# sine2pi/ASR-model

Measured on AMD Instinct MI355X. Metric: audio-sec/sec fwd+bwd on 30s@16kHz LibriSpeech-shaped clips (whole job, all GPUs), higher is better.
Workload: dtype bf16; 1 GPU; tiny (BASELINE configs[1]): log-mel + 4 enc/4 dec d=384 h=6 fwd+bwd, 32 x 30 s clips per GPU, T=256; model=tiny, global_batch=32, seq_len=3001, text_len=256, pitch_frames=3001, parallelism=dp1

## Files before the change

### asr-model_amd/asrx/gemm.py

```python
from __future__ import annotations

import torch

from . import lib, prec, probe

ACT = {"none": 0, "gelu": 1, "silu": 2, "sigmoid": 3, "relu": 4}


BF16 = torch.bfloat16


def is_bf16(t) -> bool:
    return t is not None and t.dtype == BF16


def gemm(A, B, C, *, M, N, K, lda, ldb, ldc, a_kc=True, b_kc=True, batch=1, sA=0, sB=0, sC=0,
         bias=None, Z=None, alpha=1.0, beta=0.0, act="none", conv_a=False, conv_b=False,
         conv_F=0, conv_C=0, splitk=1, precision=None):
    lib.require_gpu(A, B, C)
    if is_bf16(A) or is_bf16(B) or is_bf16(C):
        raise RuntimeError("asrx_gemm takes fp32 operands; bf16-stored activations go through the wide GEMM")
    p = prec.get() if precision is None else precision
    e0 = probe.begin("gemm")
    lib.call("asrx_gemm", p, lib.ptr(A), lda, sA, int(a_kc), int(conv_a), lib.ptr(B), ldb, sB,
# ... 237 lines not shown


def gemm_wn_rows(A, Wb, C, *, M, N, K, lda, ldc, mtiles, bias=None, alpha=1.0, beta=0.0):
    return gemm_wn(A, Wb, C, M=M, N=N, K=K, lda=lda, ldc=ldc, bias=bias, alpha=alpha, beta=beta, mtiles=mtiles)


def row_tiles(next_i, layer, L, M, device=None):
    n = int(lib.load().asrx_row_tiles_max(M))
    dev = device if device is not None else next_i.device
    tl = torch.empty(n, dtype=torch.int32, device=dev)
    cnt = torch.empty(1, dtype=torch.int32, device=dev)
    lib.call("asrx_row_tiles", lib.ptr(next_i), layer, L, M, lib.ptr(tl), lib.ptr(cnt), lib.stream())
    return tl, cnt


def linear_fwd(x, W, b=None, act="none", out=None, preact=None, wbf=None, mtiles=None, out_bf16=False):
    x2 = _rows(x)
    if not x2.is_contiguous():
        x2 = x2.contiguous()
    M, K = x2.shape
    N = W.shape[0]
    wide = use_wide(K)
    if is_bf16(x2) and not wide:
        x2 = x2.float()
    odt = BF16 if (out_bf16 and wide and N % 4 == 0) else torch.float32
    y = out if out is not None else torch.empty(*x.shape[:-1], N, device=x.device, dtype=odt)
    if wide and mtiles is not None and act == "none" and preact is None:
        gemm_wn_rows(x2, weight_bf16(W) if wbf is None else wbf, y, M=M, N=N, K=K, lda=K, ldc=N, bias=b,
                     mtiles=mtiles)
    elif use_wide(K):
        gemm_wn(x2, weight_bf16(W) if wbf is None else wbf, y, M=M, N=N, K=K, lda=K, ldc=N, bias=b, act=act,
                Z=preact)
    else:
        gemm(x2, W, y, M=M, N=N, K=K, lda=K, ldb=K, ldc=N, a_kc=True, b_kc=True, bias=b, act=act,
             Z=preact)
    return y


def linear_rot_fwd(x, W, b, m, tab, L, hd, scale, preact=None):
    x2 = _rows(x)
    if not x2.is_contiguous():
        x2 = x2.contiguous()
    M, K = x2.shape
    N = W.shape[0]
    Wb = weight_bf16(W)
    y = torch.empty(*x.shape[:-1], N, device=x.device)
    nj = _nj(M, N)
    ab = int(is_bf16(x2))
    lib.require_gpu(x2, Wb, y, m, tab)
    e0 = probe.begin("gemm")
    lib.call("asrx_gemm_wn_rot", lib.ptr(x2), ab, K, lib.ptr(Wb), Wb.stride(0), lib.ptr(y), lib.ptr(preact), N,
             lib.ptr(b), lib.ptr(m), lib.ptr(tab), L, hd, float(scale), M, N, K, nj, lib.stream())
    probe.end("gemm", e0, 2.0 * M * N * K, ("wn", M, N, K, nj, 0, "rot", preact is not None, False, ab, 0, -1))
    return y


def linear_dgrad(dy, W, out=None, beta=0.0, mtiles=None):
    """dx = dy @ W for dy (..., N), W (N, K); mtiles as in linear_fwd."""
    d2 = _rows(dy)
    if not d2.is_contiguous():
        d2 = d2.contiguous()
    M, N = d2.shape
    K = W.shape[1]
    dx = out if out is not None else torch.empty(*dy.shape[:-1], K, device=dy.device, dtype=torch.float32)
    if use_wide(N) and mtiles is not None:
        gemm_wn_rows(d2, weight_bf16(W, trans=True), dx, M=M, N=K, K=N, lda=N, ldc=K, beta=beta, mtiles=mtiles)
    elif use_wide(N):
        gemm_wn(d2, weight_bf16(W, trans=True), dx, M=M, N=K, K=N, lda=N, ldc=K, beta=beta)
    else:
        gemm(d2, W, dx, M=M, N=K, K=N, lda=N, ldb=K, ldc=K, a_kc=True, b_kc=False, beta=beta)
    return dx


def _splitk_for(m_rows: int, tiles: int) -> int:
    want = max(1, 512 // max(tiles, 1))
    return int(max(1, min(want, m_rows // 256)))


FUSED_BIAS_GRAD = True
BIAS_CHECK = None


def _staged_f32_dy(A, lda, x2, M, K, rows):
    if is_bf16(x2):
        return None if (M % 4 or K % 8 or lda % 4 or x2.stride(0) != K or A.data_ptr() % 16) else 1
    tiles = ((M + 127) // 128) * ((K + 127) // 128)
    ok4 = M % 4 == 0 and K % 4 == 0 and lda % 4 == 0 and A.data_ptr() % 16 == 0 and x2.data_ptr() % 16 == 0
    if prec.get() == prec.PREC_BF16 and ok4 and x2.stride(0) == K and (tiles <= 9 or rows <= 16384
                                                                        or (rows <= 50000 and tiles <= 72)):
        return 0
    return None


def _wgrad(A, lda, x2, out, M, K, rows, db=None):
    tiles = ((M + 127) // 128) * ((K + 127) // 128)
    sk = _splitk_for(rows, tiles)

    def staged(a_bf16, b_bf16, name, *tag):
        lib.require_gpu(A, x2, out)
        e0 = probe.begin("gemm")
        if db is not None and not FUSED_BIAS_GRAD:
            staged_db, db_ = db, None
        else:
            staged_db, db_ = None, db
        if db_ is not None:
            before = db_.clone() if BIAS_CHECK is not None else None
# ... 82 lines not shown
```

### asr-model_amd/asrx/lib.py

```python
from __future__ import annotations

import ctypes
import os

import torch

_HERE = os.path.dirname(os.path.abspath(__file__))
LIB_PATH = os.environ.get("ASRX_LIB") or os.path.join(_HERE, "libasrx.so")

_i64 = ctypes.c_int64
_i32 = ctypes.c_int
_f32 = ctypes.c_float
_p = ctypes.c_void_p
_u32 = ctypes.c_uint32

SIGNATURES = {
    "asrx_last_error": (ctypes.c_char_p, []),
    "asrx_abi_version": (_i32, []),
    "asrx_noise_hash": (_u32, [_u32, _u32]),
    "asrx_set_noise_epoch": (_i32, [_u32, _p]),
    "asrx_set_gemm_variant": (_i32, [_i32]),
    "asrx_set_attn_variant": (_i32, [_i32]),
    "asrx_set_wgrad_variant": (_i32, [_i32]),
    "asrx_mel_frames": (_i32, [_i64]),
# ... 65 lines not shown
    "asrx_axpy_row2_colsum": (_i32, [_p] * 6 + [_i64] * 3 + [_p, _i64, _p]),
    "asrx_vgate_fwd": (_i32, [_p, _p, _p, _p, _p, _p, _p, _p, _p, _p, _p, _p, _p, _i64, _i64, _i64, _f32, _p]),
    "asrx_vgate_bwd": (_i32, [_p, _p, _p, _p, _p, _p, _p, _p, _p, _p, _p, _p, _p, _p, _p, _p, _p,
                              _i64, _i64, _i64, _f32, _p]),
    "asrx_tgate_fwd": (_i32, [_p, _p, _p, _i64, _i64, _p]),
    "asrx_tgate_bwd": (_i32, [_p, _p, _p, _p, _p, _i64, _i64, _p]),
    "asrx_axpy_row": (_i32, [_p, _p, _p, _p, _i64, _i64, _p]),
    "asrx_axpy_row_bwd": (_i32, [_p, _p, _p, _p, _p, _i64, _i64, _p]),
    "asrx_axpy_row_bwd2": (_i32, [_p, _p, _p, _p, _p, _p, _i64, _i64, _p]),
    "asrx_jump_select": (_i32, [_p, _p, _p, _p, _p, _p, _p, _p, _i64, _i64, _i64, _p]),
    "asrx_jump_select_bwd": (_i32, [_p, _p, _p, _p, _p, _p, _p, _p, _p, _p, _p, _p, _i64, _i64, _i64, _p]),
    "asrx_seg_colsum": (_i32, [_p, _p, _i64, _i64, _i64, _f32, _i32, _p]),
    "asrx_msheath_ctrl_fwd": (_i32, [_p, _p, _i64, _p, _p, _p, _p, _p, _p, _i64, _i64, _i64, _i64, _i64,
                                     _p, _p, _p, _p, _p, _p, _p, _p]),
    "asrx_msheath_ctrl_bwd": (_i32, [_p, _p, _p, _p, _p, _p, _p, _p, _p, _i64, _i64, _i64, _i64, _p, _p, _p, _p, _p,
                                     _p]),
    "asrx_msheath_rec_bytes": (_i64, []),
    "asrx_msheath_ctrl_fwd2": (_i32, [_p, _p, _i64, _p, _p, _p, _i64, _p, _p, _p, _i64, _i64, _i64, _i64, _i64,
                                      _p, _p, _p, _p, _p, _p, _p, _p]),
    "asrx_msheath_ctrl_bwd2": (_i32, [_p, _p, _p, _p, _p, _p, _i64, _p, _p, _p, _i64, _i64, _i64, _i64, _p, _i32,
                                      _p, _p, _p, _p, _p, _p]),
    "asrx_jump_select4_bwd_acc": (_i32, [_p, _p, _p, _p, _p, _p, _p, _p, _p, _p, _p, _p, _p, _i64, _i64, _i64, _p]),
    "asrx_jump_bwd_part_floats": (_i64, [_i64, _i64, _i64]),
    "asrx_jump_select4_bwd_part": (_i32, [_p] * 11 + [_i64, _i64, _i64, _p]),
    "asrx_msheath_ctrl_bwd4": (_i32, [_p, _i64, _p, _p, _p, _i64, _p, _p, _p, _i64, _i64, _i64, _i64, _p, _i32]
                               + [_p] * 8),
    "asrx_axpy_row2_bwd_acc": (_i32, [_p, _p, _f32, _p, _p, _p, _p, _p, _p, _p, _p, _i64, _i64, _i64, _p]),
    "asrx_jump_select4_bwd_part2": (_i32, [_p] * 11 + [_i64, _i64, _i64, _p]),
    "asrx_jump_select4_bwd_acc2": (_i32, [_p] * 13 + [_i64, _i64, _i64, _p]),
    "asrx_axpy_row2_bwd_acc2": (_i32, [_p, _p, _p, _f32, _p, _p, _p, _p, _p, _p, _p, _p, _i64, _i64, _i64, _p]),
    "asrx_wgrad_split": (_i32, [_p, _i64, _p, _i32, _i64, _p, _i64, _p, _i64, _i64, _i64, _i64, _i64, _i64, _p]),
    "asrx_msheath_dx_final": (_i32, [_p, _p, _p, _p, _i64, _i64, _i64, _p]),
    "asrx_axpy_row2": (_i32, [_p, _p, _p, _p, _p, _i64, _i64, _p]),
    "asrx_axpy_row2_bwd": (_i32, [_p, _p, _p, _p, _p, _p, _p, _i64, _i64, _p]),
    "asrx_jump_select4": (_i32, [_p, _p, _p, _p, _p, _p, _p, _p, _i64, _i64, _i64, _p]),
    "asrx_jump_select4_bwd": (_i32, [_p, _p, _p, _p, _p, _p, _p, _p, _p, _p, _p, _p, _i64, _i64, _i64, _p]),
    "asrx_colsum": (_i32, [_p, _p, _i64, _i64, _p]),
    "asrx_add_rows": (_i32, [_p, _p, _p, _p, _i64, _i64, _i64, _p]),
    "asrx_lincomb": (_i32, [_p, _p, _p, _f32, _f32, _f32, _p, _i64, _p]),
    "asrx_act_fwd": (_i32, [_p, _p, _i64, _i32, _p]),
    "asrx_act_bwd": (_i32, [_p, _p, _p, _i64, _i32, _p]),
    "asrx_glu_fwd": (_i32, [_p, _p, _i64, _i64, _p]),
    "asrx_glu_bwd": (_i32, [_p, _p, _p, _i64, _i64, _p]),
    "asrx_dropout": (_i32, [_p, _p, _i64, _i64, _i64, _i64, _u32, _f32, _p]),
    "asrx_act_dropout_fwd": (_i32, [_p, _p, _p, _i64, _i64, _i64, _i64, _u32, _f32, _i32, _i32, _p]),
    "asrx_act_dropout_bwd": (_i32, [_p, _p, _p, _i64, _i64, _i64, _i64, _u32, _f32, _i32, _i32, _p]),
    "asrx_dwconv_fwd": (_i32, [_p, _p, _p, _p, _i64, _i64, _i64, _i64, _p]),
    "asrx_dwconv_bwd": (_i32, [_p, _p, _p, _p, _p, _p, _i64, _i64, _i64, _i64, _p]),
    "asrx_bn_fwd": (_i32, [_p, _p, _p, _p, _p, _p, _i64, _i64, _i64, _f32, _i32, _p]),
    "asrx_bn_bwd": (_i32, [_p, _p, _p, _p, _p, _p, _p, _p, _p, _p, _i64, _i64, _i64, _p]),
    "asrx_dwconv_pre_bwd": (_i32, [_p, _p, _p, _p, _p, _p, _p, _i64, _i64, _i64, _i64, _i32, _p]),
    "asrx_bn_silu_fwd": (_i32, [_p, _p, _p, _p, _p, _p, _i64, _i64, _i64, _f32, _i32, _p]),
    "asrx_bn_silu_bwd": (_i32, [_p, _p, _p, _p, _p, _p, _p, _p, _p, _p, _p, _i64, _i64, _i64, _p]),
    "asrx_stem1_fwd": (_i32, [_p, _p, _p, _p, _i64, _i64, _i64, _p]),
    "asrx_stem1_bwd": (_i32, [_p, _p, _p, _p, _i64, _i64, _i64, _p]),
    "asrx_embed_fwd": (_i32, [_p, _p, _p, _i64, _i64, _p]),
    "asrx_embed_bwd": (_i32, [_p, _p, _p, _i64, _i64, _p]),
    "asrx_ce_fwd": (_i32, [_p, _p, _p, _p, _i64, _i64, _p]),
    "asrx_ce_bwd": (_i32, [_p, _p, _p, _p, _p, _i64, _i64, _p]),
    "asrx_policy_noise": (_i32, [_p, _i64, _i64, _i64, _u32, _p]),
    "asrx_weight_to_bf16": (_i32, [_p, _p, _i64, _i64, _i64, _i32, _p]),
    "asrx_gemm_wn_router": (_i32, [_p, _i64, _p, _i64, _p, _p, _p, _i64, _p, _i64, _i64, _i64, _p]),
    "asrx_gemm_wn": (_i32, [_p, _i64, _i32, _i64, _i64, _p, _i64, _p, _i64, _p, _p, _i64, _i64, _i64, _f32, _f32,
                            _i32, _i32, _p]),
    "asrx_gemm_wn_ex": (_i32, [_p, _i32, _i64, _i32, _i64, _i64, _p, _i64, _p, _i32, _i64, _p, _p, _i64, _i64, _i64,
                               _f32, _f32, _i32, _i32, _p, _p, _p]),
    "asrx_wgrad_bf16_ex": (_i32, [_p, _i64, _p, _i32, _i64, _p, _i64, _i64, _i64, _i64, _i64, _p]),
    "asrx_abby_fwd2": (_i32, [_p, _p, _p, _p, _p, _i32, _p, _p, _i64, _i64, _i64, _i64, _i64, _u32, _i32, _p, _p, _p,
                              _p]),
    "asrx_gemm_wn_gact": (_i32, [_p, _i32, _i64, _p, _i64, _p, _p, _i64, _p, _i64, _p, _i64, _i64, _i64, _i32, _i32,
                                 _p]),
    "asrx_rotary_table": (_i32, [_p, _p, _i64, _i64, _p]),
    "asrx_rotary_fwd2": (_i32, [_p, _p, _p, _p, _p, _i64, _i64, _i64, _i64, _f32, _p]),
    "asrx_rotary_bwd2": (_i32, [_p, _p, _p, _p, _p, _p, _p, _i64, _i64, _i64, _i64, _f32, _p]),
    "asrx_abby_fwd3": (_i32, [_p, _p, _p, _p, _p, _p, _i32, _p, _p, _i64, _i64, _i64, _i64, _i64, _u32, _i32, _p, _p,
                               _p, _p, _p]),
    "asrx_abby_fwd_logits2": (_i32, [_p, _p, _p, _p, _i32, _p, _p, _i64, _i64, _i64, _i64, _i64, _u32, _i32, _p, _p,
                                     _p, _p]),
    "asrx_attn_fwd2": (_i32, [_i32, _i32, _p, _p, _p, _p, _p, _p, _p, _p, _p, _i64, _i64, _i64, _i64, _i64, _i32, _f32,
                              _p]),
    "asrx_attn_bwd2": (_i32, [_i32, _i32, _p, _p, _p, _p, _p, _p, _p, _p, _p, _p, _p, _p, _p, _p, _p, _p, _p, _p,
                              _i64, _i64, _i64, _i64, _i64, _i32, _f32, _p]),
    "asrx_small_linear_fwd2": (_i32, [_p, _i32, _p, _p, _p, _i64, _i64, _i64, _i32, _p]),
    "asrx_small_linear_bwd2": (_i32, [_p, _p, _p, _i32, _p, _p, _p, _p, _i64, _i64, _i64, _i32, _f32, _p]),
    "asrx_tgate_fwd2": (_i32, [_p, _p, _p, _i32, _i64, _i64, _p]),
    "asrx_msheath_row_fwd2": (_i32, [_p] * 6 + [_i64] + [_p] * 7 + [_i32] + [_p] * 7 + [_i64] * 4
                                    + [_f32, _f32, _p, _i64, _i64, _p]),
    "asrx_msheath_row_fwd3": (_i32, [_p] * 6 + [_i64] + [_p] * 16 + [_i64] * 4 + [_f32, _f32, _p, _i64, _i64, _p]),
    "asrx_layernorm_fwd3": (_i32, [_p, _p, _p, _p, _i32] + [_p] * 6 + [_i32, _i64, _i64, _f32, _p]),
    "asrx_jump_axpy_inplace": (_i32, [_p] * 10 + [_i64, _i64, _i64, _p]),
    "asrx_wave_pool": (_i32, [_p, _i64, _i64, _i64, _i64, _p, _p]),
    "asrx_logmel_ragged": (_i32, [_p, _i64, _i64, _i64, _p, _p, _p, _p, _p, _i32, _i64, _i64, _p, _p, _i64, _p]),
    "asrx_wave_pool_ragged": (_i32, [_p, _i64, _i64, _i64, _p, _p, _i64, _p]),
    "asrx_maxfactor_param_bytes": (_i32, []),
    "asrx_maxfactor_step": (_i32, [_p, _i32, _i64, _i64, _i64, _i64, _i64, _p, _p]),
    "asrx_maxfactor_step_ex": (_i32, [_p, _i32, _i64, _i64, _i64, _i64, _i64, _p, _p, _i32, _p]),
    "asrx_grad_stats_param_bytes": (_i32, []),
    "asrx_grad_stats": (_i32, [_p, _i32, _i64, _f32, _f32, _f32, _p, _p, _p]),
    "asrx_abby_record_cond": (_i32, [_p]),
    "asrx_gemm_wn_ce": (_i32, [_p, _i64, _p, _i64, _p, _i64, _p, _i64, _i64, _i64, _i32, _p]),
    "asrx_gemm_wn_ce_f32": (_i32, [_p, _i64, _p, _i64, _p, _i64, _p, _i64, _i64, _i64, _i32, _p]),
    "asrx_ce_part_fwd": (_i32, [_p, _i64] + [_p] * 6 + [_i64, _i64, _p]),
    "asrx_ce_part_fwd_f32": (_i32, [_p, _i64] + [_p] * 6 + [_i64, _i64, _p]),
    "asrx_gemm_wn_head": (_i32, [_p, _i64, _p, _i64, _p, _p, _p, _i64, _i64, _i64, _i32, _p]),
    "asrx_head_merge": (_i32, [_p, _i64] + [_p] * 8 + [_i64, _i64, _p]),
    "asrx_ce_bwd_bf16": (_i32, [_p] * 6 + [_i64, _i64, _p]),
# ... 107 lines not shown
```

### asr-model_amd/asrx/model.py

```python
from __future__ import annotations

import contextlib
import math

import torch
from torch import nn
from torch.nn.utils.parametrizations import weight_norm

from . import gemm as gemm_mod
from . import lib, ops, prec
from .config import Dimensions
from .noise import NoiseCtx

THETA = 30000.0

_TABLES: dict = {}


def sinusoids(ctx: int, dims: int, device) -> torch.Tensor:
    key = ("pe", ctx, dims, str(device))
    if key not in _TABLES:
        tscales = torch.exp(-torch.log(torch.tensor(float(THETA))) / (dims // 2 - 1)
                            * torch.arange(dims // 2, dtype=torch.float32))
        scaled = torch.arange(ctx, dtype=torch.float32).unsqueeze(1) * tscales.unsqueeze(0)
# ... 30 lines not shown
                 threshold: float = 0.8):
        super().__init__()
        self.size, self.alpha, self.beta, self.k, self.tx = size, alpha, beta, k, threshold
        self.mode_router = nn.Sequential(nn.Linear(dims, dims), nn.SiLU(), nn.Linear(dims, 3))

    def run(self, x, noise: NoiseCtx, site: str, sid_base: int, L: int, H: int = 1, out_bf16: bool = False,
            tgate=None, residual=None):
        return ops.abby_normal(self, x, L, H, sid_base, noise.key(site), True, out_bf16, tgate, residual)


class LayerNorm(nn.Module):

    def __init__(self, dims, eps=1e-5):
        super().__init__()
        self.dims, self.eps = dims, eps
        self.gamma = nn.Parameter(torch.ones(dims))
        self.beta = nn.Parameter(torch.zeros(dims))


def get_norm(n_type: str, dims: int):
    if n_type != "AbbyNormal":
        raise NotImplementedError(f"n_type {n_type!r}: only the reachable 'AbbyNormal' path is built "
                                  "(SURVEY.md §2 #10)")
    return AbbyNormal(dims, size=5, alpha=1e-4, beta=0.75, k=1.0, threshold=0.8)


def get_activation(act: str) -> nn.Module:
    if act != "gelu":
        raise NotImplementedError(f"act {act!r}: only 'gelu' (the configured activation) is built")
    return nn.GELU()




class ConvLite(nn.Module):
    def __init__(self, dims, kernel_size=15):
        super().__init__()
        self.point1 = nn.Conv1d(dims, dims * 2, kernel_size=1)
        self.glu = nn.GLU(dim=1)
        self.depth = nn.Conv1d(dims, dims, kernel_size=kernel_size, padding=(kernel_size - 1) // 2, groups=dims)
        self.bn = nn.BatchNorm1d(dims)
        self.swish = nn.SiLU()
        self.point2 = nn.Conv1d(dims, dims, kernel_size=1)
        self.dropout = nn.Dropout(0.1)

    def run(self, x, noise: NoiseCtx, site: str, sid_base: int):
        D = x.shape[-1]
        x = ops.fork(x)
        res = x
        y = ops.linear(x, self.point1.weight, self.point1.bias)
        y = ops.glu_dwconv(y, self.depth.weight, self.depth.bias)
        if self.training:
            stats = []
            y = ops.batch_norm_silu(y, self.bn.weight, self.bn.bias, self.bn.eps, stats)
            self._update_running(stats[0], y.shape[1])
        else:
            y = ops.batch_norm_silu_eval(y, self.bn.weight, self.bn.bias, self.bn.running_mean,
                                         self.bn.running_var, self.bn.eps)
        y = ops.linear(y, self.point2.weight, self.point2.bias)
        if self.training:
            return ops.dropout_add(res, y, sid_base, noise.key(site + ".cl"), 0.1)
        return ops.add(res, y)

    @torch.no_grad()
    def _update_running(self, stats, T):
        mean, rstd = stats
        B, C = mean.shape
        bn = self.bn
        lib.call("asrx_bn_running", lib.ptr(mean), lib.ptr(rstd), lib.ptr(bn.running_mean), lib.ptr(bn.running_var),
                 lib.ptr(bn.num_batches_tracked), B, C, T, float(bn.eps), float(bn.momentum), lib.stream())


class AudioEncoder(nn.Module):

    def __init__(self, mels, dims, head, layer, act, n_type, norm=False, enc=False):
        super().__init__()
        if norm or enc:
            raise NotImplementedError("AudioEncoder(norm/enc=True) is not reachable from Model")
        self.norm = nn.Identity()
        self.local_norm = nn.Identity()
        act_fn = get_activation(act)
        self.conv1 = nn.Sequential(nn.Conv1d(mels, dims, kernel_size=3, stride=1, padding=1), self.norm)
        self.conv2 = nn.Sequential(nn.Conv1d(1, dims, kernel_size=3, stride=1, padding=1), self.local_norm)
        self.EncoderLayer = nn.Identity()
        self.encoder = nn.ModuleList()
        for _ in range(layer):
            self.encoder.append(nn.Sequential(
                act_fn, weight_norm(nn.Conv1d(dims, dims, kernel_size=3, padding=1)),
                LayerNorm(dims),
                ConvLite(dims, kernel_size=15),
                act_fn,
                nn.Conv1d(dims, dims, kernel_size=3, stride=1, padding=1, groups=dims), act_fn, nn.Dropout(0.1)))

    def stem(self, x, out=None):
        if x.dim() == 2:
            x = x.unsqueeze(0)
        B, C, T = x.shape
        if C > 1:
            xt = x.transpose(1, 2).contiguous()
            return ops.conv3(xt, self.conv1[0], out=out)
        return ops.Stem1.apply(x.reshape(B, T), self.conv2[0].weight, self.conv2[0].bias, out)

    def layers(self, x, noise: NoiseCtx, sid_base: int):
        n = len(self.encoder)
        fused_lead = False
        for l, layer in enumerate(self.encoder):
            if not fused_lead:
                x = ops.act(x, "gelu")
            fused_lead = False
            x = ops.conv3(x, layer[1])
            x = ops.layer_norm(x, layer[2].gamma, layer[2].beta, layer[2].eps)
            x = layer[3].run(x, noise, f"enc.L{l}", sid_base)
            x = ops.act_dwconv(x, "gelu", layer[5].weight, layer[5].bias)
            if self.training:
# ... 673 lines not shown
```

### asr-model_amd/asrx/ops.py

```python
from __future__ import annotations

import ctypes
import math
import weakref

import torch

from . import decisions
from . import gemm as G
from . import lib, prec, probe

_E = torch.empty
_S = lib.stream
_P = lib.ptr


def _c(t):
    return t if t.is_contiguous() else t.contiguous()


def _rows(t):
    return t.numel() // t.shape[-1]


# ... 261 lines not shown
        ctx.set_materialize_grads(False)
        x2 = x.view(-1, x.shape[-1])
        if G.is_bf16(x2):
            raise RuntimeError("LinearRes: the residual epilogue takes an fp32 x (use ops.linear_residual)")
        M, K = x2.shape
        N = W.shape[0]
        y = _E(r.shape, device=r.device)
        Wb = G.weight_bf16(W)
        nj = G._nj(M, N)
        e0 = probe.begin("gemm")
        lib.call("asrx_gemm_wn_res", _P(x2), K, _P(Wb), Wb.stride(0), _P(y), N, _P(b), _P(r), N, M, N, K, nj, _S())
        probe.end("gemm", e0, 2.0 * M * N * K, ("wn", M, N, K, nj, 0, "none", False, True, 0, 0, -1))
        ctx.dW, ctx.db = _direct(ctx, 2, W), _direct(ctx, 3, b)
        ctx.save_for_backward(x, W, b if ctx.db else None)
        ctx.has_b = b is not None
        return y

    @staticmethod
    def backward(ctx, gy):
        x, W, b = ctx.saved_tensors
        if gy is None:
            return None, None, None, None, None
        gy = _f32(gy)
        dx = None
        if ctx.needs_input_grad[1]:
            if ctx.sink is not None:
                buf, acc = ctx.sink.target(x)
                G.linear_dgrad(gy, W, out=buf, beta=float(acc))
            else:
                dx = G.linear_dgrad(gy, W)
        dW = db = None
        gb = None
        if ctx.has_b and ctx.needs_input_grad[3]:
            gb = _gbuf(b, True) if ctx.db else torch.zeros(W.shape[0], device=gy.device)
        if ctx.needs_input_grad[2]:
            gW = _gbuf(W, ctx.dW)
            G.linear_wgrad(gy, x, out=gW, accumulate=True, db=gb)
            dW = _gret(W, gW, ctx.dW)
        elif gb is not None:
            colsum(gy, out=gb)
        if gb is not None:
            db = _gret(b, gb, ctx.db)
        return gy if ctx.needs_input_grad[0] else None, dx, dW, db, None


def linear_residual(r, x, W, b=None):
    N = W.shape[0]
    K = x.shape[-1]
    M = x.numel() // max(K, 1)
    if (prec.get() == prec.PREC_BF16 and G.use_wide(K) and N % 4 == 0 and r.dtype == torch.float32
            and x.dtype == torch.float32 and r.shape[-1] == N and x.is_cuda and G._nj(M, N) in (1, 3)):
        return LinearRes.apply(r, x, W, b, sink_of(x))
    return add(r, linear(x, W, b))


class KVProjFn(torch.autograd.Function):

    @staticmethod
    def forward(ctx, x, W, b, sink, v_bf16=False, vsink=None, src=None, rot=None, grad=False):
        x = _c(x)
        D = W.shape[0] // 2
        ctx.rot = rot is not None
        if rot is not None:
            freqs, hd, scale, ctx.src_sink, m = rot
            src = _c(src)
            L = x.shape[1]
            if m is None:
                m = _E(_rows(src), device=x.device)
                lib.call("asrx_rownorm", _P(src), _P(m), _rows(src), src.shape[-1], _S())
            tab = rotary_table(freqs, L, hd)
            kz = _E(*x.shape[:-1], D, device=x.device) if grad else None
            k = G.linear_rot_fwd(x, W[:D], b[:D], m, tab, L, hd, scale, preact=kz)
            ctx.hd, ctx.scale = hd, scale
            rsaved = (kz, src, m, freqs, tab) if grad else (None,) * 5
        else:
            k = G.linear_fwd(x, W[:D], b[:D])
            rsaved = (None,) * 5
        v = G.linear_fwd(x, W[D:], b[D:], out_bf16=v_bf16)
        ctx.vsink = vsink
        ctx.set_materialize_grads(False)
        ctx.sink = sink
        ctx.dW, ctx.db = _direct(ctx, 1, W), _direct(ctx, 2, b)
        ctx.save_for_backward(x, W, b, *rsaved)
        return k, v

    @staticmethod
    def backward(ctx, dk, dv):
        x, W, b, *rsaved = ctx.saved_tensors
        D = W.shape[0] // 2
        dk = _f32(dk)
        dv = grad_in(dv, ctx.vsink)
        dsrc = None
        if ctx.rot and dk is not None and rsaved[1] is not None:
            dk, dsrc = _rotary_bwd(ctx, dk, *rsaved, ctx.needs_input_grad[6], ctx.src_sink)
        if dk is not None:
            dk = dk.reshape(*x.shape[:-1], D)
        if dv is not None:
            dv = dv.reshape(*x.shape[:-1], D)
        dx = None
        if ctx.needs_input_grad[0]:
            if ctx.sink is not None:
                buf, acc = ctx.sink.target(x)
            else:
                buf, acc = _E(x.shape, device=x.device), 0
            for gpart, Wp in ((dk, W[:D]), (dv, W[D:])):
                if gpart is not None:
# ... 1008 lines not shown
        x, w, b = ctx.saved_tensors
        g = _c(g)
        B, T, C = x.shape
        K = w.shape[-1]
        dx = _E(x.shape, device=x.device)
        dw, db = _gbuf(w, ctx.dw), _gbuf(b, ctx.db)
        lib.call("asrx_dwconv_bwd", _P(g), _P(x), _P(w), _P(dx), _P(dw), _P(db), B, T, C, K, _S())
        return dx, _gret(w, dw, ctx.dw), _gret(b, db, ctx.db)


class BatchNormPS(torch.autograd.Function):

    @staticmethod
    def forward(ctx, x, w, b, eps, stats):
        x = _c(x)
        B, T, C = x.shape
        mean = _E(B, C, device=x.device)
        rstd = _E(B, C, device=x.device)
        y = _E(x.shape, device=x.device)
        lib.call("asrx_bn_fwd", _P(x), _P(w), _P(b), _P(y), _P(mean), _P(rstd), B, T, C, float(eps), 1, _S())
        if stats is not None:
            stats.append((mean, rstd))
        ctx.dw, ctx.db = _direct(ctx, 1, w), _direct(ctx, 2, b)
        ctx.save_for_backward(x, w, mean, rstd, b)
        return y

    @staticmethod
    def backward(ctx, g):
        x, w, mean, rstd, b = ctx.saved_tensors
        g = _c(g)
        B, T, C = x.shape
        sg = _E(B, C, device=x.device)
        sgx = _E(B, C, device=x.device)
        dx = _E(x.shape, device=x.device)
        dw, db = _gbuf(w, ctx.dw), _gbuf(b, ctx.db)
        lib.call("asrx_bn_bwd", _P(g), _P(x), _P(mean), _P(rstd), _P(w), _P(sg), _P(sgx), _P(dx), _P(dw), _P(db), B,
                 T, C, _S())
        return dx, _gret(w, dw, ctx.dw), _gret(b, db, ctx.db), None, None


def batch_norm_eval(x, w, b, rm, rv, eps):
    x = _c(x)
    B, T, C = x.shape
    rstd = _E(rv.shape, device=x.device)
    lib.call("asrx_rsqrt_eps", _P(_c(rv)), _P(rstd), rv.numel(), float(eps), _S())
    y = _E(x.shape, device=x.device)
    lib.call("asrx_bn_fwd", _P(x), _P(w), _P(b), _P(y), _P(_c(rm)), _P(rstd), B, T, C, float(eps), 0, _S())
    return y


FUSED_ENCODER = True
DW_PRE = {"glu": 1, "gelu": 2}
_DW_PRE_K = {"glu": 15, "gelu": 3}


def _aligned(t):
    t = _c(t)
    return t if t.data_ptr() % 16 == 0 else t.clone()


class PreDWConv(torch.autograd.Function):

    @staticmethod
    def forward(ctx, z, w, b, pre):
        z = _c(z)
        B, T = z.shape[:2]
        C, K = w.shape[0], w.shape[-1]
        if z.dim() != 3 or z.shape[-1] != (2 * C if pre == "glu" else C):
            raise ValueError(f"PreDWConv({pre}): input {tuple(z.shape)} does not match {C} conv channels")
        x = _E(B, T, C, device=z.device)
        if pre == "glu":
            lib.call("asrx_glu_fwd", _P(z), _P(x), B * T, C, _S())
        else:
            lib.call("asrx_act_fwd", _P(z), _P(x), x.numel(), ACT[pre], _S())
        y = _E(B, T, C, device=z.device)
        lib.call("asrx_dwconv_fwd", _P(x), _P(w), _P(b), _P(y), B, T, C, K, _S())
        ctx.pre = pre
        ctx.dw, ctx.db = _direct(ctx, 1, w), _direct(ctx, 2, b)
        ctx.save_for_backward(z, x, w, b)
        return y

    @staticmethod
    def backward(ctx, g):
        z, x, w, b = ctx.saved_tensors
        g = _aligned(g)
        B, T, C = x.shape
        K = w.shape[-1]
        dz = _E(z.shape, device=z.device)
        dw, db = _gbuf(w, ctx.dw), _gbuf(b, ctx.db)
        lib.call("asrx_dwconv_pre_bwd", _P(g), _P(x), _P(z), _P(w), _P(dz), _P(dw), _P(db), B, T, C, K,
                 DW_PRE[ctx.pre], _S())
        return dz, _gret(w, dw, ctx.dw), _gret(b, db, ctx.db), None


def _pre_dwconv(z, w, pre):
    C, K = w.shape[0], w.shape[-1]
    return (FUSED_ENCODER and K == _DW_PRE_K[pre] and C % 4 == 0 and z.numel() < 1 << 31
            and z.data_ptr() % 16 == 0)


def glu_dwconv(x, w, b):
    x = _c(x)
    if _pre_dwconv(x, w, "glu"):
        return PreDWConv.apply(x, w, b, "glu")
    return DWConv.apply(glu(x), w, b)


def act_dwconv(x, name, w, b):
    x = _c(x)
    if name == "gelu" and _pre_dwconv(x, w, "gelu"):
        return PreDWConv.apply(x, w, b, "gelu")
    return DWConv.apply(act(x, name), w, b)


class BatchNormSiLU(torch.autograd.Function):

    @staticmethod
    def forward(ctx, x, w, b, eps, stats):
        x = _c(x)
        B, T, C = x.shape
        mean = _E(B, C, device=x.device)
        rstd = _E(B, C, device=x.device)
        y = _E(x.shape, device=x.device)
        lib.call("asrx_bn_silu_fwd", _P(x), _P(w), _P(b), _P(y), _P(mean), _P(rstd), B, T, C, float(eps), 1, _S())
        if stats is not None:
            stats.append((mean, rstd))
        ctx.dw, ctx.db = _direct(ctx, 1, w), _direct(ctx, 2, b)
        ctx.save_for_backward(x, w, mean, rstd, b)
        return y

    @staticmethod
    def backward(ctx, g):
        x, w, mean, rstd, b = ctx.saved_tensors
        g = _aligned(g)
        B, T, C = x.shape
        sg = _E(B, C, device=x.device)
        sgx = _E(B, C, device=x.device)
        dx = _E(x.shape, device=x.device)
        dw, db = _gbuf(w, ctx.dw), _gbuf(b, ctx.db)
        lib.call("asrx_bn_silu_bwd", _P(g), _P(x), _P(mean), _P(rstd), _P(w), _P(b), _P(sg), _P(sgx), _P(dx), _P(dw),
                 _P(db), B, T, C, _S())
        return dx, _gret(w, dw, ctx.dw), _gret(b, db, ctx.db), None, None


def _bn_silu_ok(x, *ps):
    return (FUSED_ENCODER and x.shape[-1] % 4 == 0 and x.numel() < 1 << 31
            and all(t.data_ptr() % 16 == 0 for t in (x,) + ps))


def batch_norm_silu(x, w, b, eps, stats):
    x = _c(x)
    if _bn_silu_ok(x, w, b):
        return BatchNormSiLU.apply(x, w, b, eps, stats)
    return act(BatchNormPS.apply(x, w, b, eps, stats), "silu")


def batch_norm_silu_eval(x, w, b, rm, rv, eps):
    x, rm = _c(x), _c(rm)
    if not _bn_silu_ok(x, w, b, rm):
        return act(batch_norm_eval(x, w, b, rm, rv, eps), "silu")
    B, T, C = x.shape
    rstd = _E(rv.shape, device=x.device)
    lib.call("asrx_rsqrt_eps", _P(_c(rv)), _P(rstd), rv.numel(), float(eps), _S())
    y = _E(x.shape, device=x.device)
    lib.call("asrx_bn_silu_fwd", _P(x), _P(w), _P(b), _P(y), _P(rm), _P(rstd), B, T, C, float(eps), 0, _S())
    return y


class Conv3(torch.autograd.Function):

    @staticmethod
    def forward(ctx, x, g, v, b, out=None):
        x = _c(x)
        B, T, Ci = x.shape
        Co = v.shape[0]
        dev = x.device
        nrm = _E(Co, device=dev) if g is not None else None
        wide = G.use_wide(3 * Ci)
        Wt = None if wide else _E(Co, 3 * Ci, device=dev)
        Wtb = _E(Co, 3 * Ci, dtype=torch.int16, device=dev) if wide else None
        lib.call("asrx_conv3_weight", _P(g), _P(_c(v)), Co, Ci, _P(Wt), _P(Wtb), None, None, _P(nrm), _S())
        y = _E(B, T, Co, device=dev) if out is None else out
        if wide:
            G.gemm_wn(x, Wtb, y, M=B * T, N=Co, K=3 * Ci, lda=Ci, ldc=Co, bias=b, conv=True, conv_F=T, conv_C=Ci)
        else:
            G.gemm(x, Wt, y, M=B * T, N=Co, K=3 * Ci, lda=Ci, ldb=3 * Ci, ldc=Co, bias=b, conv_a=True, conv_F=T,
                   conv_C=Ci)
        ctx.has_g = g is not None
        ctx.dg = _direct(ctx, 1, g) if g is not None else False
        ctx.dv, ctx.db = _direct(ctx, 2, v), _direct(ctx, 3, b)
        ctx.save_for_backward(x, g, v, b, nrm)
        return y

    @staticmethod
    def backward(ctx, gy):
        x, g, v, b, nrm = ctx.saved_tensors
        gy = _c(gy)
        B, T, Ci = x.shape
        Co = v.shape[0]
        dev = x.device
        v = _c(v)
        dx = None
        if ctx.needs_input_grad[0]:
            wide = G.use_wide(3 * Co)
            Wf = None if wide else _E(Ci, 3 * Co, device=dev)
            Wfb = _E(Ci, 3 * Co, dtype=torch.int16, device=dev) if wide else None
# ... 287 lines not shown
```

### asr-model_amd/csrc/common.h

```cpp
#pragma once
#include <hip/hip_runtime.h>
#include <stdint.h>
#include <string>
#include <cstdio>
#include <cstdarg>

typedef __attribute__((ext_vector_type(8))) __bf16 bf16x8;
typedef __attribute__((ext_vector_type(4))) float f32x4;
typedef __attribute__((ext_vector_type(16))) float f32x16;

namespace asrx {

enum Prec : int { PREC_F32 = 0, PREC_BF16 = 1, PREC_X3 = 3 };

enum Act : int { ACT_NONE = 0, ACT_GELU = 1, ACT_SILU = 2, ACT_SIGMOID = 3, ACT_RELU = 4 };
constexpr int ACT_SOFTMAX = 16;

void set_error(const char* fmt, ...);
int check_launch(const char* what);

}

#define ASRX_NOISE_EPOCH_SETTER(NAME)                                                                      \
  extern "C" int NAME(uint32_t epoch, hipStream_t stream) {                                               \
// ... 178 lines not shown
}
__device__ __forceinline__ void glds16(const void* gsrc, uint32_t lds_dst) {
  unsigned keep;
  asm volatile("s_mov_b32 %0, m0\n\ts_mov_b32 m0, %2\n\ts_nop 0\n\tglobal_load_lds_dwordx4 %1, off\n\ts_mov_b32 m0, %0"
               : "=&s"(keep) : "v"(gsrc), "s"(lds_dst) : "memory");
}
__device__ __forceinline__ void glds4(const void* gsrc, uint32_t lds_dst) {
  unsigned keep;
  asm volatile("s_mov_b32 %0, m0\n\ts_mov_b32 m0, %2\n\ts_nop 0\n\tglobal_load_lds_dword %1, off\n\ts_mov_b32 m0, %0"
               : "=&s"(keep) : "v"(gsrc), "s"(lds_dst) : "memory");
}
__device__ __forceinline__ void wait_vm_le(int n) {
  if (n >= 48) asm volatile("s_waitcnt vmcnt(48)" ::: "memory");
  else if (n >= 40) asm volatile("s_waitcnt vmcnt(40)" ::: "memory");
  else if (n >= 32) asm volatile("s_waitcnt vmcnt(32)" ::: "memory");
  else if (n >= 28) asm volatile("s_waitcnt vmcnt(28)" ::: "memory");
  else if (n >= 24) asm volatile("s_waitcnt vmcnt(24)" ::: "memory");
  else if (n >= 20) asm volatile("s_waitcnt vmcnt(20)" ::: "memory");
  else if (n >= 16) asm volatile("s_waitcnt vmcnt(16)" ::: "memory");
  else if (n >= 12) asm volatile("s_waitcnt vmcnt(12)" ::: "memory");
  else if (n >= 10) asm volatile("s_waitcnt vmcnt(10)" ::: "memory");
  else if (n >= 8) asm volatile("s_waitcnt vmcnt(8)" ::: "memory");
  else if (n >= 6) asm volatile("s_waitcnt vmcnt(6)" ::: "memory");
  else if (n >= 5) asm volatile("s_waitcnt vmcnt(5)" ::: "memory");
  else if (n >= 4) asm volatile("s_waitcnt vmcnt(4)" ::: "memory");
  else if (n >= 3) asm volatile("s_waitcnt vmcnt(3)" ::: "memory");
  else if (n >= 2) asm volatile("s_waitcnt vmcnt(2)" ::: "memory");
  else if (n >= 1) asm volatile("s_waitcnt vmcnt(1)" ::: "memory");
  else asm volatile("s_waitcnt vmcnt(0)" ::: "memory");
}

__host__ __device__ __forceinline__ int float_to_ordered(float f) {
  int i = __builtin_bit_cast(int, f);
  return i >= 0 ? i : i ^ 0x7fffffff;
}
__host__ __device__ __forceinline__ float ordered_to_float(int i) {
  return __builtin_bit_cast(float, i >= 0 ? i : i ^ 0x7fffffff);
}

__host__ __device__ __forceinline__ uint32_t mix32(uint32_t x) {
  x ^= x >> 16;
  x *= 0x7feb352dU;
  x ^= x >> 15;
  x *= 0x846ca68bU;
  x ^= x >> 16;
  return x;
}
static __device__ uint32_t g_noise_epoch;
__device__ __forceinline__ uint32_t noise_key(uint32_t key) {
  const uint32_t ep = *(const __attribute__((address_space(4))) uint32_t*)&g_noise_epoch;
  if (ep != 0u) key ^= mix32(ep * 0x9E3779B9U + 0x7F4A7C15U);
  return key;
}
__device__ __forceinline__ float noise_uniform_k(uint32_t key, uint32_t idx) {
  uint32_t h = mix32(mix32(idx ^ key) + (key * 0x9E3779B9U + 0x632BE5ABU));
  return ((float)(h >> 9) + 0.5f) * (1.0f / 8388608.0f);
}
__device__ __forceinline__ float noise_uniform(uint32_t key, uint32_t idx) {
  return noise_uniform_k(noise_key(key), idx);
}
__device__ __forceinline__ float noise_gumbel_k(uint32_t key, uint32_t idx) {
  float u = noise_uniform_k(key, idx);
  return -logf(-logf(u));
}
__device__ __forceinline__ float noise_gumbel(uint32_t key, uint32_t idx) { return noise_gumbel_k(noise_key(key), idx); }

}

#define ASRX_NOISE_EPOCH_SETTER(NAME)                                                                      \
  extern "C" int NAME(uint32_t epoch, hipStream_t stream) {                                               \
    static uint32_t host_epoch[64];                                                                       \
    static unsigned slot = 0;                                                                             \
    uint32_t* src = &host_epoch[(slot++) & 63];     \
    *src = epoch;                                                                                         \
    hipError_t e = hipMemcpyToSymbolAsync(HIP_SYMBOL(asrx::g_noise_epoch), src, sizeof(uint32_t), 0,      \
                                          hipMemcpyHostToDevice, stream);                                 \
    if (e != hipSuccess) {                                                                                \
      asrx::set_error("%s: %s", #NAME, hipGetErrorString(e));                                             \
      return (int)e;                                                                                      \
    }                                                                                                     \
    return 0;                                                                                             \
  }
```

### asr-model_amd/csrc/gemm_p2.h

```cpp
#pragma once
#include "gemm_wr.h"

namespace asrx {
namespace wn {

namespace p2 {
constexpr int NT2 = 256;
constexpr int WNC = 2;

template <int NJ, bool ABF>
struct Geo {
  static constexpr int BN = WNC * 32 * NJ;
  static constexpr int ACH = BM * BK * (ABF ? 2 : 4) / 16 / NT2;
  static constexpr int WCH = BN * BK * 2 / 16 / NT2;
  static_assert(BM * BK * (ABF ? 2 : 4) % (16 * NT2) == 0 && BN * BK * 2 % (16 * NT2) == 0, "chunking");
};

template <int NJ, bool ABF>
struct Stage {
  u32x4 a[Geo<NJ, ABF>::ACH];
  u32x4 b[Geo<NJ, ABF>::WCH];
};

template <int NJ, bool ABF>
// ... 37 lines not shown
    const int q = t + NT2 * i;
    const int n = min(n0 + (q >> 2), p.N - 1);
    o.w[i] = (uint32_t)(((int64_t)n * p.ldw + 8 * (q & 3)) * 2);
  }
}
template <int NJ, bool ABF>
__device__ __forceinline__ void load_fast(const Params& p, Stage<NJ, ABF>& st, const Off<NJ, ABF>& o, int k0) {
  const char* A = reinterpret_cast<const char*>(p.A) + (size_t)k0 * (ABF ? 2 : 4);
  const char* W = reinterpret_cast<const char*>(p.W) + (size_t)k0 * 2;
#pragma unroll
  for (int i = 0; i < Geo<NJ, ABF>::ACH; ++i) st.a[i] = *reinterpret_cast<const u32x4*>(A + o.a[i]);
#pragma unroll
  for (int i = 0; i < Geo<NJ, ABF>::WCH; ++i) st.b[i] = *reinterpret_cast<const u32x4*>(W + o.w[i]);
}

template <int NJ, bool ABF>
__device__ __forceinline__ void store(const Stage<NJ, ABF>& st, char* At, char* Bt) {
  const int t = threadIdx.x;
#pragma unroll
  for (int i = 0; i < Geo<NJ, ABF>::ACH; ++i) {
    const int q = t + NT2 * i;
    if constexpr (ABF) {
      const int row = q >> 2, c = q & 3;
      *reinterpret_cast<u32x4*>(At + row * 64 + 16 * (c ^ swb(row))) = st.a[i];
    } else {
      const int row = q >> 3, c = q & 7;
      const float4 v = __builtin_bit_cast(float4, st.a[i]);
      typedef __attribute__((ext_vector_type(4))) __bf16 bf16x4;
      bf16x4 h;
      h[0] = (__bf16)v.x; h[1] = (__bf16)v.y; h[2] = (__bf16)v.z; h[3] = (__bf16)v.w;
      *reinterpret_cast<bf16x4*>(At + row * 64 + 16 * ((c >> 1) ^ swb(row)) + 8 * (c & 1)) = h;
    }
  }
#pragma unroll
  for (int i = 0; i < Geo<NJ, ABF>::WCH; ++i) {
    const int q = t + NT2 * i;
    const int n = q >> 2, c = q & 3;
    *reinterpret_cast<u32x4*>(Bt + n * 64 + 16 * (c ^ swb(n))) = st.b[i];
  }
}
}

#ifndef P2_ABL
#define P2_ABL 0
#endif
#ifndef P2_FAST
#define P2_FAST 1
#endif
#ifndef P2_DEPTH
#define P2_DEPTH 3
#endif

constexpr bool p2_built(int nj, bool abf, Epi e) {
  return e == Epi::Plain ? nj == 2 || nj == 3 : e == Epi::Res ? nj == 3 && !abf : e == Epi::Rot && nj == 3;
}

template <int NJ, bool ABF, int ACT, Epi EPI>
__global__ __launch_bounds__(p2::NT2, 2) void gemm_p2_kernel(Params p, int ntiles) {
  static_assert(p2_built(NJ, ABF, EPI), "not a gemm_p2_kernel instantiation (p2_built)");
  static_assert(EPI == Epi::Plain || ACT == ACT_NONE, "the residual and rotary epilogues take no activation");
  using namespace p2;
  typedef Geo<NJ, ABF> GE;
  constexpr int BN = GE::BN, NT = 2 * NJ;
  constexpr int AB = BM * BK * 2, BB = BN * BK * 2;
  __shared__ __attribute__((aligned(16))) char a_img[2][AB];
  __shared__ __attribute__((aligned(16))) char b_img[2][BB];
  __shared__ __attribute__((aligned(16))) float bias_s[2][BN];
  __shared__ __attribute__((aligned(16))) float ep_s[4 * EpLds<NJ>::FLOATS];

  const int nN = (p.N + BN - 1) / BN;
  const int nk = (p.K + BK - 1) / BK;
  const int G = gridDim.x, bid = blockIdx.x;
  const int r = (G % 8 == 0) ? (bid & 7) * (G >> 3) + (bid >> 3) : bid;
  const int* mlist = p.mtiles;
  if (mlist) ntiles = *p.n_mtiles * nN;
  const int my = r < ntiles ? (ntiles - r + G - 1) / G : 0;
  const int S = my * nk;
  float* ep = ep_s + (threadIdx.x >> 6) * EpLds<NJ>::FLOATS;
  const int wid = threadIdx.x >> 6, lane = threadIdx.x & 63;
  const int wm = wid >> 1, wn = wid & 1;
  const int lr = lane & 15, lk = lane >> 4;

  struct Cur {
    int j, kk, m0, n0;
  };
  auto enter = [&](Cur& c) __attribute__((always_inline)) {
    const int t = c.j * G + r;
    const int tm = t / nN;
    c.m0 = ((mlist && t < ntiles) ? ((const __attribute__((address_space(4))) int*)mlist)[tm] : tm) * BM;
    c.n0 = (t - tm * nN) * BN;
  };
  auto advance = [&](Cur& c) __attribute__((always_inline)) {
    if (++c.kk == nk) {
      c.kk = 0;
      ++c.j;
      enter(c);
    }
  };
  Cur cl{0, 0, 0, 0}, cs{0, 0, 0, 0}, ce{0, 0, 0, 0};
  enter(cl);
  cs = cl;
  ce = cl;
  typedef Stage<NJ, ABF> Stg;
  const bool fast = P2_FAST && (ABF || NJ < 3) && p.K % BK == 0 && (uint64_t)p.M * p.lda * (ABF ? 2 : 4) < (1ull << 32) &&
                    (uint64_t)p.N * p.ldw * 2 < (1ull << 32);
  Off<NJ, ABF> off;
  auto ld = [&](Stg& st) __attribute__((always_inline)) {
    if (fast) {
      if (cl.kk == 0) offsets<NJ, ABF>(p, off, cl.m0, cl.n0);
      load_fast<NJ, ABF>(p, st, off, cl.kk * BK);
    } else {
      load<NJ, ABF>(p, st, cl.m0, cl.n0, cl.kk * BK);
    }
// ... 84 lines not shown
  }
}

template <int NJ, bool ABF, int ACT, Epi EPI>
void launch_p2(const Params& p, hipStream_t s) {
  static int resident = 0;
  const void* fn = (const void*)gemm_p2_kernel<NJ, ABF, ACT, EPI>;
  if (!resident) {
    int per_cu = 0, dev = 0, cus = 0;
    (void)hipOccupancyMaxActiveBlocksPerMultiprocessor(&per_cu, fn, p2::NT2, 0);
    (void)hipGetDevice(&dev);
    (void)hipDeviceGetAttribute(&cus, hipDeviceAttributeMultiprocessorCount, dev);
    resident = std::max(1, per_cu) * std::max(1, cus);
  }
  const int tiles = ((p.M + BM - 1) / BM) * ((p.N + p2::Geo<NJ, ABF>::BN - 1) / p2::Geo<NJ, ABF>::BN);
  const int grid = std::min(tiles, resident);
  gemm_p2_kernel<NJ, ABF, ACT, EPI><<<grid, p2::NT2, 0, s>>>(p, tiles);
}

template <int NJ, bool ABF, Epi EPI>
void launch_p2_act(const Params& p, hipStream_t s) {
  if constexpr (EPI != Epi::Plain) {
    launch_p2<NJ, ABF, ACT_NONE, EPI>(p, s);
  } else {
    switch (p.act) {
      case ACT_GELU: launch_p2<NJ, ABF, ACT_GELU, EPI>(p, s); break;
      case ACT_SILU: launch_p2<NJ, ABF, ACT_SILU, EPI>(p, s); break;
      case ACT_SIGMOID: launch_p2<NJ, ABF, ACT_SIGMOID, EPI>(p, s); break;
      case ACT_RELU: launch_p2<NJ, ABF, ACT_RELU, EPI>(p, s); break;
      default: launch_p2<NJ, ABF, ACT_NONE, EPI>(p, s); break;
    }
  }
}

}
}

#ifdef ASRX_P2_INSTANTIATE
#define ASRX_P2_EXTERN
#else
#define ASRX_P2_EXTERN extern
#endif
#define ASRX_P2_INST(NJ, ABF, EPI)                                                               \
  ASRX_P2_EXTERN template void asrx::wn::launch_p2_act<NJ, asrx::wn::ABF, asrx::wn::Epi::EPI>( \
      const asrx::wn::Params&, hipStream_t);
#ifndef ASRX_P2_INSTANTIATE
ASRX_P2_INST(3, BF16A, Rot)
ASRX_P2_INST(3, F32A, Rot)
ASRX_P2_INST(3, F32A, Plain)
ASRX_P2_INST(3, BF16A, Plain)
ASRX_P2_INST(2, F32A, Plain)
ASRX_P2_INST(2, BF16A, Plain)
ASRX_P2_INST(3, F32A, Res)
#endif
```

### asr-model_amd/csrc/gemm_wn.hip

```cpp
#include "gemm_wr.h"
#include "gemm_p2.h"
#include "gemm_ws.h"
#include <string>

static int g_wide_variant = 5;
extern "C" int asrx_set_gemm_variant(int v) {
  const int old = g_wide_variant;
  g_wide_variant = v;
  return old;
}

enum class WideKernel { WS, P2, WR };
static WideKernel wide_kernel(const asrx::wn::Params& p, asrx::wn::Epi epi, int conv, int nj, int a_bf16) {
  const int v = g_wide_variant;
  if ((v & 4) != 0 && !conv && asrx::wn::ws_ok(p, a_bf16, (v & 8) != 0)) return WideKernel::WS;
  const bool vec = ((p.N | p.ldc) & 3) == 0 && ((uintptr_t)p.C & 15) == 0 && ((uintptr_t)p.Z & 15) == 0 &&
                   ((uintptr_t)p.Cb & 7) == 0;
  const bool width = epi == asrx::wn::Epi::Plain ? nj == 3 || nj == 2 || (nj == 1 && (v & 3) == 2) : nj == 3;
  if ((a_bf16 || p.M < 131072) && (v & 3) >= 1 && !conv && width && vec && p.K >= 64) return WideKernel::P2;
  return WideKernel::WR;
}

namespace asrx {
namespace wn {
// ... 177 lines not shown
  wn::Params p = wide_params(A, lda, W, ldw, nullptr, ldc, nullptr, nullptr, M, N, K);
  p.Cb = Zb;
  p.ce_part = (float2*)part;
  p.ce_ld = (int)((N + 128 * nj - 1) / (128 * nj));
  return launched(run_wr<wn::Epi::CE>(p, 0, nj, 1, stream), "asrx_gemm_wn_ce");
}

extern "C" int asrx_gemm_wn_ce_f32(const void* A, int64_t lda, const unsigned short* W, int64_t ldw, float* Zf,
                               int64_t ldc, float* part, int64_t M, int64_t N, int64_t K, int nj, hipStream_t stream) {
  if (int rc = wide_check("asrx_gemm_wn_ce_f32", A, 1, lda, W, ldw, M, N, K,
                          {((uintptr_t)Zf & 15) == 0 && ((uintptr_t)part & 7) == 0,
                           "A/W 16-byte, Zf 16-byte, part 8-byte aligned"},
                          {N % 4 == 0 && ldc % 4 == 0, "K, lda, ldw % 8 and N, ldc % 4 required"}))
    return rc;
  ASRX_REQUIRE(nj >= 1 && nj <= 3, "asrx_gemm_wn_ce_f32: nj in 1..3");
  wn::Params p = wide_params(A, lda, W, ldw, Zf, ldc, nullptr, nullptr, M, N, K);
  p.ce_part = (float2*)part;
  p.ce_ld = (int)((N + 128 * nj - 1) / (128 * nj));
  return launched(run_wr<wn::Epi::CE>(p, 0, nj, 1, stream), "asrx_gemm_wn_ce_f32");
}

extern "C" int asrx_gemm_wn_head(const void* A, int64_t lda, const unsigned short* W, int64_t ldw, float* part,
                                 const int64_t* labels, float* zlab, int64_t M, int64_t N, int64_t K, int nj,
                                 hipStream_t stream) {
  if (int rc = wide_check("asrx_gemm_wn_head", A, 1, lda, W, ldw, M, N, K,
                          {((uintptr_t)part & 7) == 0, "A/W 16-byte, part 8-byte aligned"},
                          {N % 4 == 0 && lda >= K, "K, lda, ldw % 8, N % 4 and lda >= K required"}))
    return rc;
  ASRX_REQUIRE(nj >= 1 && nj <= 3, "asrx_gemm_wn_head: nj in 1..3");
  ASRX_REQUIRE(!labels || zlab, "asrx_gemm_wn_head: labels need zlab");
  const int64_t nparts = (N + 128 * nj - 1) / (128 * nj);
  wn::Params p = wide_params(A, lda, W, ldw, nullptr, N, nullptr, nullptr, M, N, K);
  p.ce_part = (float2*)part;
  p.ce_ld = (int)nparts;
  p.hd_idx = reinterpret_cast<int*>(part + 2 * M * nparts);
  p.hd_labels = labels;
  p.hd_zlab = zlab;
  return launched(run_wr<wn::Epi::Head>(p, 0, nj, 1, stream), "asrx_gemm_wn_head");
}

extern "C" int asrx_gemm_wn_res(const float* A, int64_t lda, const unsigned short* W, int64_t ldw, float* C, int64_t ldc,
                                const float* bias, const float* R, int64_t ldr, int64_t M, int64_t N, int64_t K, int nj,
                                hipStream_t stream) {
  if (int rc = wide_check("asrx_gemm_wn_res", A, 0, lda, W, ldw, M, N, K,
                          {((uintptr_t)C & 15) == 0 && ((uintptr_t)R & 15) == 0, "A/W/C/R must be 16-byte aligned"},
                          {N % 4 == 0 && ldc % 4 == 0 && ldr % 4 == 0, "K, ldw % 8; lda, N, ldc, ldr % 4"}))
    return rc;
  ASRX_REQUIRE(R && R != C, "asrx_gemm_wn_res: a residual input distinct from C is required");
  ASRX_REQUIRE(nj == 1 || nj == 3, "asrx_gemm_wn_res: nj 1 or 3");
  wn::Params p = wide_params(A, lda, W, ldw, C, ldc, bias, nullptr, M, N, K);
  p.Rres = R;
  p.ldr = (int)ldr;
  return launched(run_wide<wn::Epi::Res>(p, 0, nj, 0, stream), "asrx_gemm_wn_res");
}

extern "C" int asrx_gemm_wn_rot(const void* A, int a_bf16, int64_t lda, const unsigned short* W, int64_t ldw,
                                float* C, float* Z, int64_t ldc, const float* bias, const float* m, const float* tab,
                                int64_t L, int64_t hd, float scale, int64_t M, int64_t N, int64_t K, int nj,
                                hipStream_t stream) {
  const bool heads = hd >= 4 && hd % 4 == 0 && N % hd == 0;
  if (int rc = wide_check("asrx_gemm_wn_rot", A, a_bf16, lda, W, ldw, M, N, K,
                          {((uintptr_t)C & 15) == 0 && ((uintptr_t)Z & 15) == 0 && ((uintptr_t)tab & 15) == 0,
                           "A/W/C/Z/tab must be 16-byte aligned"},
                          {N % 4 == 0 && ldc % 4 == 0, "K, ldw % 8; lda % 4 (8 bf16); N, ldc % 4"},
                          L > 0 ? nullptr : "empty problem", heads ? nullptr : "head dim % 4, N % hd"))
    return rc;
  ASRX_REQUIRE(m && tab, "asrx_gemm_wn_rot: row norms and angle table required");
  ASRX_REQUIRE(nj == 1 || nj == 3, "asrx_gemm_wn_rot: nj 1 or 3");
  wn::Params p = wide_params(A, lda, W, ldw, C, ldc, bias, Z, M, N, K);
  p.rot_m = m;
  p.rot_tab = reinterpret_cast<const float2*>(tab);
  p.rot_L = (int)L;
  p.rot_half = (int)(hd / 2);
  p.rot_scale = scale;
  return launched(run_wide<wn::Epi::Rot>(p, 0, nj, a_bf16, stream), "asrx_gemm_wn_rot");
}

extern "C" int asrx_gemm_wn_gact(const void* A, int a_bf16, int64_t lda, const unsigned short* W, int64_t ldw,
                                 const float* bias, const float* G, int64_t ldg, unsigned short* gz, int64_t ldc,
                                 float* db, int64_t M, int64_t N, int64_t K, int act, int nj, hipStream_t stream) {
  const char* early = nj != 3 ? "nj 3 only"
                      : act != ACT_GELU && act != ACT_SILU && act != ACT_SIGMOID ? "gelu/silu/sigmoid only" : nullptr;
  if (int rc = wide_check("asrx_gemm_wn_gact", A, a_bf16, lda, W, ldw, M, N, K,
                          {((uintptr_t)G & 15) == 0 && ((uintptr_t)gz & 7) == 0, "A/W/G 16-byte, gz 8-byte aligned"},
                          {N % 4 == 0 && ldc % 4 == 0 && ldg % 4 == 0, "K, ldw % 8; lda % 4 (8 bf16); N, ldc, ldg % 4"},
                          early))
    return rc;
  wn::Params p = wide_params(A, lda, W, ldw, nullptr, ldc, bias, nullptr, M, N, K, 1.f, 0.f, act);
  p.Cb = gz;
  p.G = G;
  p.ldg = (int)ldg;
  p.dB = db;
  return launched(run_wr<wn::Epi::GAct>(p, 0, nj, a_bf16, stream), "asrx_gemm_wn_gact");
}

extern "C" int asrx_gemm_wn_rows(const float* A, int64_t lda, const unsigned short* W, int64_t ldw, float* C,
                                 int64_t ldc, const float* bias, float* Z, int64_t M, int64_t N, int64_t K,
                                 float alpha, float beta, int act, int nj, const int* mtiles, const int* n_mtiles,
                                 hipStream_t stream) {
  if (int rc = wide_check("asrx_gemm_wn_rows", A, 0, lda, W, ldw, M, N, K)) return rc;
  ASRX_REQUIRE(mtiles && n_mtiles, "asrx_gemm_wn_rows: tile list required");
  wn::Params p = wide_params(A, lda, W, ldw, C, ldc, bias, Z, M, N, K, alpha, beta, act);
  p.mtiles = mtiles;
  p.n_mtiles = n_mtiles;
  return launched(run_wr<wn::Epi::Plain>(p, 0, nj, 0, stream), "asrx_gemm_wn_rows");
}
// ... 181 lines not shown
```

### asr-model_amd/csrc/gemm_wr.h

```cpp
#pragma once
#include "common.h"

namespace asrx {

namespace wn {

constexpr int BM = 128, BK = 32, NTHR = 512;
constexpr int A_BYTES = BM * BK * 4;

static __device__ __attribute__((aligned(16))) float zero_page[4];

enum class Epi {
  Plain,
  Router,
  CE,
  Head,
  Res,
  GAct,
  Rot
};
constexpr bool ROWS = false, CONV3 = true;
constexpr bool F32A = false, BF16A = true;

struct Params {
  const float* A;
  int lda;
  const unsigned short* W;
  int ldw;
  float* C;
  int ldc;
  const float* bias;
  float* Z;
  int M, N, K;
  int convF, convC;
  float alpha, beta;
  int act;
  const float* W2;
  float* R;
  const int* mtiles;
  const int* n_mtiles;
  unsigned short* Cb;
  float2* ce_part;
  int ce_ld;
  const float* Rres;
  int ldr;
  const float* G;
  int ldg;
  float* dB;
  const float* rot_m;
  const float2* rot_tab;
  int rot_L, rot_half;
  float rot_scale;
  int* hd_idx;
  const int64_t* hd_labels;
  float* hd_zlab;
};

__device__ __forceinline__ void st_bf16x4(unsigned short* dst, float a, float b, float c, float d) {
  typedef __attribute__((ext_vector_type(4))) __bf16 bf16x4;
  const bf16x4 h = {(__bf16)a, (__bf16)b, (__bf16)c, (__bf16)d};
  __builtin_nontemporal_store(__builtin_bit_cast(unsigned long long, h), reinterpret_cast<unsigned long long*>(dst));
}

template <int NJ>
struct Cfg {
  static constexpr int BN = 128 * NJ;
  static constexpr int B_BYTES = BN * BK * 2;
  static constexpr int STAGE = A_BYTES + B_BYTES;
  static constexpr int PIECES = 2 + NJ;
  static constexpr int BNR = (BN + NTHR - 1) / NTHR * NTHR;
  static constexpr int BIAS_OPS = BNR / NTHR;
};

__device__ __forceinline__ int swa(int row) { return ((row >> 1) & 1) | (((row >> 3) & 1) << 2); }
__device__ __forceinline__ int swb(int n) { return ((n >> 3) & 1) << 1; }

__device__ __forceinline__ bool vec_ok(const Params& p) {
  return ((p.N | p.ldc) & 3) == 0 && ((uintptr_t)p.C & 15) == 0 && ((uintptr_t)p.Z & 15) == 0 &&
         ((uintptr_t)p.Cb & 7) == 0;
}

template <int ACT>
__device__ __forceinline__ float act_t(float x) {
  if constexpr (ACT == ACT_GELU) return gelu_f(x);
  else if constexpr (ACT == ACT_SILU) return silu_f(x);
  else if constexpr (ACT == ACT_SIGMOID) return sigmoid_f(x);
  else if constexpr (ACT == ACT_RELU) return x > 0.f ? x : 0.f;
  else return x;
}

template <int NJ, int ACT>
__device__ __forceinline__ void epilogue(const Params& p, f32x4 (&acc)[4][2 * NJ], const float* bsl, int m0, int n0,
                                         int wm, int wn, int lr, int lk) {
  constexpr int NT = 2 * NJ;
  const bool vec = vec_ok(p);
#pragma unroll
  for (int nt = 0; nt < NT; ++nt) {
    const int nl = wn * (32 * NJ) + nt * 16 + 4 * lk;
// ... 12 lines not shown
      if (p.Cb) {
        unsigned short* hd = p.Cb + (int64_t)row * p.ldc + col;
#pragma unroll
        for (int r = 0; r < 4; ++r) {
          if (col + r >= p.N) break;
          if (zdst) zdst[r] = v[r];
          hd[r] = __builtin_bit_cast(unsigned short, (__bf16)act_t<ACT>(v[r]));
        }
        continue;
      }
      if (vec) {
        if (p.beta != 0.f) {
          const float4 o = *reinterpret_cast<const float4*>(dst);
          v[0] += p.beta * o.x; v[1] += p.beta * o.y; v[2] += p.beta * o.z; v[3] += p.beta * o.w;
        }

        if (zdst) __builtin_nontemporal_store(f32x4{v[0], v[1], v[2], v[3]}, reinterpret_cast<f32x4*>(zdst));
        __builtin_nontemporal_store(f32x4{act_t<ACT>(v[0]), act_t<ACT>(v[1]), act_t<ACT>(v[2]), act_t<ACT>(v[3])},
                                    reinterpret_cast<f32x4*>(dst));
      } else {
#pragma unroll
        for (int r = 0; r < 4; ++r) {
          if (col + r >= p.N) break;
          float x = v[r];
          if (p.beta != 0.f) x += p.beta * dst[r];
          if (zdst) zdst[r] = x;
          dst[r] = act_t<ACT>(x);
        }
      }
    }
  }
}

#ifndef WR_ABL_EPI
#define WR_ABL_EPI 0
#endif
constexpr int EP_PAD = 4;
template <int NJ>
struct EpLds {
  static constexpr int W = 32 * NJ;
  static constexpr int LD = W + EP_PAD;
  static constexpr int FLOATS = 16 * LD;
};
__device__ __forceinline__ float4 rot_apply(const Params& p, float4 x, int row, int col) {
#pragma clang fp contract(off)
  const int hd = 2 * p.rot_half;
  const int j = (col % hd) >> 1;
  const float4 t = *reinterpret_cast<const float4*>(p.rot_tab + (int64_t)(row % p.rot_L) * p.rot_half + j);
  const float mm = p.rot_m[row] * p.rot_scale;
  return make_float4(mm * (x.x * t.x - x.y * t.y), mm * (x.x * t.y + x.y * t.x), mm * (x.z * t.z - x.w * t.w),
                     mm * (x.z * t.w + x.w * t.z));
}

template <int NJ, int ACT, Epi EPI = Epi::Plain>
__device__ __forceinline__ void epilogue_lds(const Params& p, f32x4 (&acc)[4][2 * NJ], const float* bsl, int m0,
                                             int n0, int wm, int wn, int lr, int lk, float* ep) {
  constexpr bool RES = EPI == Epi::Res, ROT = EPI == Epi::Rot;
  static_assert(EPI == Epi::Plain || ((RES || ROT) && ACT == ACT_NONE), "plain, or residual / rotary without activation");
  constexpr int NT = 2 * NJ, W = EpLds<NJ>::W, LD = EpLds<NJ>::LD, W4 = W / 4;
  constexpr int PER = 16 * W4 / 64;
  static_assert((16 * W4) % 64 == 0, "slice must split evenly over the wave");
  const int lane = threadIdx.x & 63;
  const int cbase = n0 + wn * W;
#pragma unroll
  for (int mt = 0; mt < 4; ++mt) {
#pragma unroll
    for (int nt = 0; nt < NT; ++nt) {
      const int nl = nt * 16 + 4 * lk;
      float4 bv = make_float4(0.f, 0.f, 0.f, 0.f);
      if (p.bias) bv = *reinterpret_cast<const float4*>(bsl + wn * W + nl);
      *reinterpret_cast<float4*>(ep + lr * LD + nl) =
          make_float4(p.alpha * acc[mt][nt][0] + bv.x, p.alpha * acc[mt][nt][1] + bv.y,
                      p.alpha * acc[mt][nt][2] + bv.z, p.alpha * acc[mt][nt][3] + bv.w);
    }
    __builtin_amdgcn_wave_barrier();
    const int rbase = m0 + wm * 64 + mt * 16;
#pragma unroll
    for (int j = 0; j < PER; ++j) {
      const int f = j * 64 + lane, r = f / W4, c = 4 * (f % W4);
      float4 x = *reinterpret_cast<const float4*>(ep + r * LD + c);
      const int row = rbase + r, col = cbase + c;
      if (row >= p.M || col >= p.N) continue;
#if WR_ABL_EPI == 2
      if (x.x + x.y + x.z + x.w != 1.2345e-37f) continue;
#endif
      if (p.Cb) {
        if (p.Z)
          __builtin_nontemporal_store(f32x4{x.x, x.y, x.z, x.w},
                                      reinterpret_cast<f32x4*>(p.Z + (int64_t)row * p.ldc + col));
        st_bf16x4(p.Cb + (int64_t)row * p.ldc + col, act_t<ACT>(x.x), act_t<ACT>(x.y), act_t<ACT>(x.z),
                  act_t<ACT>(x.w));
        continue;
      }
      float* dst = p.C + (int64_t)row * p.ldc + col;
      if (p.beta != 0.f) {
        const float4 o = *reinterpret_cast<const float4*>(dst);
        x.x += p.beta * o.x; x.y += p.beta * o.y; x.z += p.beta * o.z; x.w += p.beta * o.w;
      }
      if constexpr (RES) {
        const float4 o = *reinterpret_cast<const float4*>(p.Rres + (int64_t)row * p.ldr + col);
        x.x += o.x; x.y += o.y; x.z += o.z; x.w += o.w;
      }
      if (p.Z)
        __builtin_nontemporal_store(f32x4{x.x, x.y, x.z, x.w},
                                    reinterpret_cast<f32x4*>(p.Z + (int64_t)row * p.ldc + col));
      if constexpr (ROT) x = rot_apply(p, x, row, col);
      __builtin_nontemporal_store(f32x4{act_t<ACT>(x.x), act_t<ACT>(x.y), act_t<ACT>(x.z), act_t<ACT>(x.w)},
                                  reinterpret_cast<f32x4*>(dst));
    }
    __builtin_amdgcn_wave_barrier();
  }
}

template <int ACT>
__device__ __forceinline__ float dact_t(float v) {
  if constexpr (ACT == ACT_GELU) return gelu_grad(v);
  else if constexpr (ACT == ACT_SILU) return silu_grad(v);
  else {
    const float sg = sigmoid_f(v);
    return sg * (1.f - sg);
  }
}
template <int NJ, int ACT>
__device__ __forceinline__ void epilogue_gact(const Params& p, f32x4 (&acc)[4][2 * NJ], const float* bsl, int m0,
                                              int n0, int wm, int wn, int lr, int lk, float* ep) {
  constexpr int NT = 2 * NJ, W = EpLds<NJ>::W, LD = EpLds<NJ>::LD, W4 = W / 4;
  constexpr int PER = 16 * W4 / 64;
  constexpr int CS = (W + 63) / 64;
  const int lane = threadIdx.x & 63;
  const int cbase = n0 + wn * W;
  float csum[CS];
#pragma unroll
  for (int i = 0; i < CS; ++i) csum[i] = 0.f;
#pragma unroll
  for (int mt = 0; mt < 4; ++mt) {
#pragma unroll
    for (int nt = 0; nt < NT; ++nt) {
      const int nl = nt * 16 + 4 * lk;
      float4 bv = make_float4(0.f, 0.f, 0.f, 0.f);
      if (p.bias) bv = *reinterpret_cast<const float4*>(bsl + wn * W + nl);
      *reinterpret_cast<float4*>(ep + lr * LD + nl) =
          make_float4(p.alpha * acc[mt][nt][0] + bv.x, p.alpha * acc[mt][nt][1] + bv.y,
                      p.alpha * acc[mt][nt][2] + bv.z, p.alpha * acc[mt][nt][3] + bv.w);
    }
    __builtin_amdgcn_wave_barrier();
    const int rbase = m0 + wm * 64 + mt * 16;
#pragma unroll
    for (int j = 0; j < PER; ++j) {
      const int f = j * 64 + lane, r = f / W4, c = 4 * (f % W4);
      float* sl = ep + r * LD + c;
      const float4 z = *reinterpret_cast<const float4*>(sl);
      const int row = rbase + r, col = cbase + c;
      float4 o = make_float4(0.f, 0.f, 0.f, 0.f);
      if (row < p.M && col < p.N) {
        const float4 g = *reinterpret_cast<const float4*>(p.G + (int64_t)row * p.ldg + col);
        o = make_float4(g.x * dact_t<ACT>(z.x), g.y * dact_t<ACT>(z.y), g.z * dact_t<ACT>(z.z),
                        g.w * dact_t<ACT>(z.w));
        st_bf16x4(p.Cb + (int64_t)row * p.ldc + col, o.x, o.y, o.z, o.w);
      }
// ... 434 lines not shown
    const int n = q >> 3, c = q & 7;
    *reinterpret_cast<u32x4*>(Bt + n * 128 + 16 * (c ^ sw64(n))) = st.b[i];
  }
}

template <bool ABF>
struct WrOff64 {
  uint32_t a[ABF ? 2 : 4];
  uint32_t w[2];
};
template <bool ABF>
__device__ __forceinline__ void wr_offsets64(const Params& p, WrOff64<ABF>& o, int m0, int n0) {
  const int t = threadIdx.x;
#pragma unroll
  for (int i = 0; i < (ABF ? 2 : 4); ++i) {
    const int q = t + NTHR * i;
    if constexpr (ABF) {
      const int row = min(m0 + (q >> 3), p.M - 1);
      o.a[i] = (uint32_t)(((int64_t)row * p.lda + 8 * (q & 7)) * 2);
    } else {
      const int row = min(m0 + (q >> 4), p.M - 1);
      o.a[i] = (uint32_t)(((int64_t)row * p.lda + 4 * (q & 15)) * 4);
    }
  }
#pragma unroll
  for (int i = 0; i < 2; ++i) {
    const int q = t + NTHR * i;
    const int n = min(n0 + (q >> 3), p.N - 1);
    o.w[i] = (uint32_t)(((int64_t)n * p.ldw + 8 * (q & 7)) * 2);
  }
}
template <bool ABF>
__device__ __forceinline__ void wr_load64_fast(const Params& p, WrStage64<ABF>& st, const WrOff64<ABF>& o, uint32_t ka,
                                               uint32_t kw) {
  const char* A = reinterpret_cast<const char*>(p.A);
  const char* W = reinterpret_cast<const char*>(p.W);
#pragma unroll
  for (int i = 0; i < (ABF ? 2 : 4); ++i) {
    if constexpr (ABF) st.a[i] = *reinterpret_cast<const u32x4*>(A + (o.a[i] + ka));
    else st.a[i] = *reinterpret_cast<const float4*>(A + (o.a[i] + ka));
  }
#pragma unroll
  for (int i = 0; i < 2; ++i) st.b[i] = *reinterpret_cast<const u32x4*>(W + (o.w[i] + kw));
}

constexpr bool wr_built(int nj, bool conv, bool abf, Epi e) {
  if (nj < 1 || nj > 3) return false;
  switch (e) {
    case Epi::Plain: return true;
    case Epi::Router: return !conv && !abf;
    case Epi::CE: return !conv && abf;
    case Epi::Head: return !conv && abf;
    case Epi::Res: return !conv && !abf && nj != 2;
    case Epi::GAct: return !conv && nj == 3;
    case Epi::Rot: return !conv && nj != 2;
  }
  return false;
}

template <int NJ, bool CONV, bool ABF, Epi EPI>
__global__ __launch_bounds__(NTHR, 1) void gemm_wr_kernel(Params p, int ntiles) {
  constexpr bool RT = EPI == Epi::Router, HEAD = EPI == Epi::Head, CE = EPI == Epi::CE || HEAD;
  constexpr bool RES = EPI == Epi::Res, GA = EPI == Epi::GAct, ROT = EPI == Epi::Rot;
  static_assert(!HEAD || (CE && ABF), "the head epilogue is a variant of the bf16-A CE instantiation");
  static_assert(wr_built(NJ, CONV, ABF, EPI), "not a gemm_wr_kernel instantiation (wr_built)");
  typedef Cfg<NJ> CF;
  constexpr int BN = CF::BN, NT = 2 * NJ, BNR = CF::BNR;
  constexpr bool K64 = NJ == 1 && !CONV;
  constexpr int BKW = K64 ? 64 : BK;
  typedef typename pick_t<K64, WrStage64<ABF>, WrStage<NJ, ABF>>::type Stg;
  constexpr int AB = BM * BKW * 2, BB = BN * BKW * 2;
  __shared__ __attribute__((aligned(16))) char a_img[2][AB];
  __shared__ __attribute__((aligned(16))) char b_img[2][BB];
  __shared__ __attribute__((aligned(16))) float bias_s[2][BNR];
  __shared__ float w2s[RT ? 3 * BN : 1];
  __shared__ __attribute__((aligned(16))) float red[RT ? BM * 12 : (CE ? BM * 8 : 1)];
  __shared__ int redi[HEAD ? BM * 4 : 1];
  __shared__ int lab_s[HEAD ? 2 * BM : 1];
  __shared__ __attribute__((aligned(16))) float ep_s[RT ? 1 : 8 * EpLds<NJ>::FLOATS];
  if constexpr (RT) {
    for (int i = threadIdx.x; i < 3 * BN; i += NTHR) {
      const int k = i / BN, n = i % BN;
      w2s[i] = n < p.N ? p.W2[k * p.N + n] : 0.f;
    }
  }

  const int nN = (p.N + BN - 1) / BN;
  const int nk = (p.K + BKW - 1) / BKW;
  const int G = gridDim.x, bid = blockIdx.x;
  const int r = (G % 8 == 0) ? (bid & 7) * (G >> 3) + (bid >> 3) : bid;
  const int* mlist = p.mtiles;
  if (mlist) ntiles = *p.n_mtiles * nN;
  const int my = r < ntiles ? (ntiles - r + G - 1) / G : 0;
  const int S = my * nk;
  float* ep = ep_s + (threadIdx.x >> 6) * EpLds<NJ>::FLOATS;
  const int wid = threadIdx.x >> 6, lane = threadIdx.x & 63;
  const int wm = wid >> 2, wn = wid & 3;
  const int lr = lane & 15, lk = lane >> 4;
  const bool vec = vec_ok(p);

  struct Cur {
    int j, kk, m0, n0;
  };
  auto enter = [&](Cur& c) __attribute__((always_inline)) {
    const int t = c.j * G + r;
    if constexpr (CE) {
      const int nM = (p.M + BM - 1) / BM;
      c.m0 = (t < ntiles ? t % nM : nM + t) * BM;
      c.n0 = (t < ntiles ? t / nM : 0) * BN;
    } else {
      const int tm = t / nN;
      c.m0 = ((mlist && t < ntiles) ? ((const __attribute__((address_space(4))) int*)mlist)[tm] : tm) * BM;
      c.n0 = (t - tm * nN) * BN;
    }
  };
  auto advance = [&](Cur& c) __attribute__((always_inline)) {
// ... 82 lines not shown
          b[nt] = *reinterpret_cast<const bf16x8*>(Bt + n * 128 + 16 * ((4 * h + lk) ^ sw64(n)));
        }
#pragma unroll
        for (int mt = 0; mt < 4; ++mt)
#pragma unroll
          for (int nt = 0; nt < NT; ++nt)
            acc[mt][nt] = __builtin_amdgcn_mfma_f32_16x16x32_bf16(b[nt], a[mt], acc[mt][nt], 0, 0, 0);
      }
    } else {
      bf16x8 a[4], b[NT];
#pragma unroll
      for (int mt = 0; mt < 4; ++mt) {
        const int rr = wm * 64 + mt * 16 + lr;
        a[mt] = *reinterpret_cast<const bf16x8*>(At + rr * 64 + 16 * (lk ^ swb(rr)));
      }
#pragma unroll
      for (int nt = 0; nt < NT; ++nt) {
        const int n = wn * (32 * NJ) + nt * 16 + lr;
        b[nt] = *reinterpret_cast<const bf16x8*>(Bt + n * 64 + 16 * (lk ^ swb(n)));
      }
#pragma unroll
      for (int mt = 0; mt < 4; ++mt)
#pragma unroll
        for (int nt = 0; nt < NT; ++nt)
          acc[mt][nt] = __builtin_amdgcn_mfma_f32_16x16x32_bf16(b[nt], a[mt], acc[mt][nt], 0, 0, 0);
    }
    if (s + 1 < S) store(s + 1, nxt);
    if (ce.kk == nk - 1) {
      const int m0 = ce.m0, n0 = ce.n0;
      const float* bsl = bias_s[ce.j & 1];
#if WR_ABL_EPI == 1
      {
        float t = 0.f;
#pragma unroll
        for (int i = 0; i < 4; ++i)
#pragma unroll
          for (int q = 0; q < NT; ++q) t += acc[i][q][0] + acc[i][q][1] + acc[i][q][2] + acc[i][q][3];
        if (t == 1.2345e-37f) p.C[m0] = t;
      }
      if constexpr (true) {
      } else
#endif
      if constexpr (RT) {
        epilogue_router<NJ>(p, acc, bsl, w2s, red, m0, wm, wn, lr, lk);
      } else if constexpr (HEAD) {
        epilogue_head<NJ>(p, acc, m0, n0, wm, wn, lr, lk, ep, reinterpret_cast<float2*>(red), redi,
                          lab_s + (ce.j & 1) * BM);
      } else if constexpr (CE) {
        epilogue_ce<NJ>(p, acc, m0, n0, wm, wn, lr, lk, ep, reinterpret_cast<float2*>(red));
      } else if constexpr (RES) {
        epilogue_lds<NJ, ACT_NONE, Epi::Res>(p, acc, bsl, m0, n0, wm, wn, lr, lk, ep);
      } else if constexpr (ROT) {
        epilogue_lds<NJ, ACT_NONE, Epi::Rot>(p, acc, bsl, m0, n0, wm, wn, lr, lk, ep);
      } else if constexpr (GA) {
        switch (p.act) {
          case ACT_GELU: epilogue_gact<NJ, ACT_GELU>(p, acc, bsl, m0, n0, wm, wn, lr, lk, ep); break;
          case ACT_SILU: epilogue_gact<NJ, ACT_SILU>(p, acc, bsl, m0, n0, wm, wn, lr, lk, ep); break;
          default: epilogue_gact<NJ, ACT_SIGMOID>(p, acc, bsl, m0, n0, wm, wn, lr, lk, ep); break;
        }
      } else if (WR_EPI_LDS && vec) switch (p.act) {
        case ACT_GELU: epilogue_lds<NJ, ACT_GELU>(p, acc, bsl, m0, n0, wm, wn, lr, lk, ep); break;
        case ACT_SILU: epilogue_lds<NJ, ACT_SILU>(p, acc, bsl, m0, n0, wm, wn, lr, lk, ep); break;
        case ACT_SIGMOID: epilogue_lds<NJ, ACT_SIGMOID>(p, acc, bsl, m0, n0, wm, wn, lr, lk, ep); break;
        case ACT_RELU: epilogue_lds<NJ, ACT_RELU>(p, acc, bsl, m0, n0, wm, wn, lr, lk, ep); break;
        default: epilogue_lds<NJ, ACT_NONE>(p, acc, bsl, m0, n0, wm, wn, lr, lk, ep); break;
      } else switch (p.act) {
        case ACT_GELU: epilogue<NJ, ACT_GELU>(p, acc, bsl, m0, n0, wm, wn, lr, lk); break;
        case ACT_SILU: epilogue<NJ, ACT_SILU>(p, acc, bsl, m0, n0, wm, wn, lr, lk); break;
        case ACT_SIGMOID: epilogue<NJ, ACT_SIGMOID>(p, acc, bsl, m0, n0, wm, wn, lr, lk); break;
        case ACT_RELU: epilogue<NJ, ACT_RELU>(p, acc, bsl, m0, n0, wm, wn, lr, lk); break;
        default: epilogue<NJ, ACT_NONE>(p, acc, bsl, m0, n0, wm, wn, lr, lk); break;
      }
#pragma unroll
      for (int i = 0; i < 4; ++i)
#pragma unroll
        for (int q = 0; q < NT; ++q) acc[i][q] = f32x4{0.f, 0.f, 0.f, 0.f};
    }
    advance(ce);
    __syncthreads();
  };

  for (int s = 0; s < S; s += DEPTH) {
    if constexpr (DEPTH == 3) {
      kstep(s, st0, st1);
      if (s + 1 < S) kstep(s + 1, st1, st2);
      if (s + 2 < S) kstep(s + 2, st2, st0);
    } else if constexpr (DEPTH == 4) {
      kstep(s, st0, st1);
      if (s + 1 < S) kstep(s + 1, st1, st2);
      if (s + 2 < S) kstep(s + 2, st2, st3);
      if (s + 3 < S) kstep(s + 3, st3, st0);
    } else {
      kstep(s, st0, st1);
      if (s + 1 < S) kstep(s + 1, st1, st2);
      if (s + 2 < S) kstep(s + 2, st2, st3);
      if (s + 3 < S) kstep(s + 3, st3, st4);
      if (s + 4 < S) kstep(s + 4, st4, st0);
    }
  }
}

template <int NJ, bool CONV, bool ABF, Epi EPI>
void launch_wr(const Params& p, hipStream_t s) {
  static int resident = 0;
  const void* fn = (const void*)gemm_wr_kernel<NJ, CONV, ABF, EPI>;
  if (!resident) {
    int per_cu = 0, dev = 0, cus = 0;
    (void)hipOccupancyMaxActiveBlocksPerMultiprocessor(&per_cu, fn, NTHR, 0);
    (void)hipGetDevice(&dev);
    (void)hipDeviceGetAttribute(&cus, hipDeviceAttributeMultiprocessorCount, dev);
    resident = std::max(1, per_cu) * std::max(1, cus);
  }
  const int tiles = ((p.M + BM - 1) / BM) * ((p.N + Cfg<NJ>::BN - 1) / Cfg<NJ>::BN);
  const int grid = std::min(tiles, resident);
  gemm_wr_kernel<NJ, CONV, ABF, EPI><<<grid, NTHR, 0, s>>>(p, tiles);
}

}
}

#ifdef ASRX_WR_INSTANTIATE
#define ASRX_WR_EXTERN
#else
#define ASRX_WR_EXTERN extern
#endif
#define ASRX_WR_INST(NJ, CONV, ABF, EPI)                                                                    \
  ASRX_WR_EXTERN template void asrx::wn::launch_wr<NJ, asrx::wn::CONV, asrx::wn::ABF, asrx::wn::Epi::EPI>( \
      const asrx::wn::Params&, hipStream_t);
#define ASRX_WR_SET(NJ)                                                                                  \
  ASRX_WR_INST(NJ, ROWS, F32A, Plain) ASRX_WR_INST(NJ, CONV3, F32A, Plain) ASRX_WR_INST(NJ, ROWS, BF16A, Plain) \
  ASRX_WR_INST(NJ, CONV3, BF16A, Plain) ASRX_WR_INST(NJ, ROWS, F32A, Router)
#ifndef ASRX_WR_INSTANTIATE
ASRX_WR_SET(1)
ASRX_WR_SET(2)
ASRX_WR_SET(3)
ASRX_WR_INST(1, ROWS, BF16A, CE)
ASRX_WR_INST(2, ROWS, BF16A, CE)
ASRX_WR_INST(3, ROWS, BF16A, CE)
ASRX_WR_INST(1, ROWS, F32A, Res)
ASRX_WR_INST(3, ROWS, F32A, Res)
ASRX_WR_INST(3, ROWS, F32A, GAct)
ASRX_WR_INST(3, ROWS, BF16A, GAct)
ASRX_WR_INST(1, ROWS, BF16A, Rot)
ASRX_WR_INST(1, ROWS, F32A, Rot)
ASRX_WR_INST(3, ROWS, BF16A, Rot)
ASRX_WR_INST(3, ROWS, F32A, Rot)
ASRX_WR_INST(1, ROWS, BF16A, Head)
ASRX_WR_INST(2, ROWS, BF16A, Head)
ASRX_WR_INST(3, ROWS, BF16A, Head)
#endif
```

### asr-model_amd/csrc/gemm_ws.h

```cpp
#pragma once
#include "gemm_wr.h"

namespace asrx {
namespace wn {
namespace ws {

constexpr int BN = 128;
constexpr int KMAX = 384;
constexpr int ROWB = KMAX * 2;
constexpr int WTHR = 512;
template <bool ABF>
struct WsCfg {
  static constexpr int KS = ABF ? 32 : 64;
  static constexpr int CH = KS / 8;
  static constexpr bool PIPE = ABF;
  static constexpr int NBUF = PIPE ? 3 : 2;
  static constexpr int DEPTH = ABF ? 6 : 4;
};
template <int KS>
__device__ __forceinline__ int aswz(int row) {
  if constexpr (KS == 64) return sw64(row);
  else return swb(row);
}

__device__ __forceinline__ int wchunk(int n, int c) { return (c & ~15) | ((c ^ n) & 15); }

template <bool ABF>
struct Stage {
  static constexpr int NA = ABF ? WsCfg<ABF>::KS / 32 : WsCfg<ABF>::KS / 16;
  u32x4 a[NA];
};

template <bool ABF>
__device__ __forceinline__ void stage_store(const Stage<ABF>& st, char* At) {
  constexpr int KS = WsCfg<ABF>::KS, CH = WsCfg<ABF>::CH;
  const int t = threadIdx.x;
#pragma unroll
  for (int i = 0; i < Stage<ABF>::NA; ++i) {
    const int q = t + WTHR * i;
    if constexpr (ABF) {
      const int row = q / CH, c = q % CH;
      *reinterpret_cast<u32x4*>(At + row * (2 * KS) + 16 * (c ^ aswz<KS>(row))) = st.a[i];
    } else {
      const int row = q / (2 * CH), c = q % (2 * CH);
      const float4 v = __builtin_bit_cast(float4, st.a[i]);
      typedef __attribute__((ext_vector_type(4))) __bf16 bf16x4;
      bf16x4 h;
      h[0] = (__bf16)v.x; h[1] = (__bf16)v.y; h[2] = (__bf16)v.z; h[3] = (__bf16)v.w;
      *reinterpret_cast<bf16x4*>(At + row * (2 * KS) + 16 * ((c >> 1) ^ aswz<KS>(row)) + 8 * (c & 1)) = h;
    }
  }
}

}

constexpr bool ws_built(bool abf, Epi e) { return e == Epi::Plain || e == Epi::Rot || (e == Epi::Res && !abf); }

template <bool ABF, int ACT, Epi EPI>
__global__ __launch_bounds__(ws::WTHR, 1) void gemm_ws_kernel(Params p, int nS, int lanes) {
  static_assert(ws_built(ABF, EPI), "not a gemm_ws_kernel instantiation (ws_built)");
  static_assert(EPI == Epi::Plain || ACT == ACT_NONE, "the residual and rotary epilogues take no activation");
  using namespace ws;
  constexpr int KS = WsCfg<ABF>::KS, CH = WsCfg<ABF>::CH, NBUF = WsCfg<ABF>::NBUF, DEPTH = WsCfg<ABF>::DEPTH;
  constexpr bool PIPE = WsCfg<ABF>::PIPE;
  __shared__ __attribute__((aligned(16))) char w_img[BN * ROWB];
  __shared__ __attribute__((aligned(16))) char a_img[NBUF][BM * KS * 2];
  __shared__ __attribute__((aligned(16))) float bias_s[BN];
  __shared__ __attribute__((aligned(16))) float ep_s[8 * EpLds<1>::FLOATS];

  const int G = gridDim.x;
  int r;
  {
    const int per = G / 8, rem = G % 8, x = blockIdx.x % 8, q = blockIdx.x / 8;
    r = (x < rem ? x * (per + 1) : rem * (per + 1) + (x - rem) * per) + q;
  }
  const int s = r % nS, lane0 = r / nS;
  const int n0 = s * BN;
  const int nM = (p.M + BM - 1) / BM;
  const int my = lane0 < nM ? (nM - lane0 + lanes - 1) / lanes : 0;
  const int nk = p.K / KS;
  const int S = my * nk;
  const int tid = threadIdx.x, wid = tid >> 6, lane = tid & 63;
  const int wm = wid >> 2, wn = wid & 3;
  const int lr = lane & 15, lk = lane >> 4;
  float* ep = ep_s + wid * EpLds<1>::FLOATS;

  {
    const int nch = p.K / 8;
    for (int i = tid; i < BN * nch; i += WTHR) {
      const int n = i / nch, c = i - n * nch;
      u32x4 v = {0u, 0u, 0u, 0u};
      if (n0 + n < p.N) v = *reinterpret_cast<const u32x4*>(p.W + (int64_t)(n0 + n) * p.ldw + 8 * c);
      *reinterpret_cast<u32x4*>(w_img + n * ROWB + 16 * wchunk(n, c)) = v;
    }
    for (int c = tid; c < BN; c += WTHR) bias_s[c] = (p.bias && n0 + c < p.N) ? p.bias[n0 + c] : 0.f;
  }

  constexpr int AES = ABF ? 2 : 4;
  int lj = 0, lkk = 0;
  constexpr int NA = Stage<ABF>::NA, CE = ABF ? CH : 2 * CH, EL = ABF ? 8 : 4;
  const char *ab0 = nullptr, *ab1 = nullptr, *ab2 = nullptr, *ab3 = nullptr;
  auto enter = [&]() __attribute__((always_inline)) {
    const int m0 = (lane0 + lj * lanes) * BM;
    const char* A = reinterpret_cast<const char*>(p.A);
    auto at = [&](int i) __attribute__((always_inline)) {
      const int q = tid + WTHR * i;
      return A + ((int64_t)min(m0 + q / CE, p.M - 1) * p.lda + EL * (q % CE)) * AES;
    };
    ab0 = at(0);
// ... 164 lines not shown

inline bool ws_ok(const Params& p, bool a_bf16, bool any_shape = false) {
  const bool vec = ((p.N | p.ldc) & 3) == 0 && ((uintptr_t)p.C & 15) == 0 && ((uintptr_t)p.Z & 15) == 0 &&
                   ((uintptr_t)p.Cb & 7) == 0;
  return vec && !p.mtiles && p.K % (a_bf16 ? ws::WsCfg<true>::KS : ws::WsCfg<false>::KS) == 0 &&
         p.K <= ws::KMAX && p.M >= 32768 && ((p.N + ws::BN - 1) / ws::BN) <= 64 &&
         (any_shape || (a_bf16 ? p.N >= 768 : p.N <= 768));
}

template <bool ABF, int ACT, Epi EPI>
void launch_ws(const Params& p, hipStream_t s) {
  static int cus = 0;
  if (!cus) {
    int dev = 0;
    (void)hipGetDevice(&dev);
    (void)hipDeviceGetAttribute(&cus, hipDeviceAttributeMultiprocessorCount, dev);
    cus = std::max(1, cus);
  }
  const int nS = (p.N + ws::BN - 1) / ws::BN;
  const int nM = (p.M + BM - 1) / BM;
  const int lanes = std::max(1, std::min(cus / nS, nM));
  gemm_ws_kernel<ABF, ACT, EPI><<<nS * lanes, ws::WTHR, 0, s>>>(p, nS, lanes);
}

template <bool ABF, Epi EPI>
void launch_ws_act(const Params& p, hipStream_t s) {
  if constexpr (EPI != Epi::Plain) {
    launch_ws<ABF, ACT_NONE, EPI>(p, s);
  } else {
    switch (p.act) {
      case ACT_GELU: launch_ws<ABF, ACT_GELU, EPI>(p, s); break;
      case ACT_SILU: launch_ws<ABF, ACT_SILU, EPI>(p, s); break;
      case ACT_SIGMOID: launch_ws<ABF, ACT_SIGMOID, EPI>(p, s); break;
      case ACT_RELU: launch_ws<ABF, ACT_RELU, EPI>(p, s); break;
      default: launch_ws<ABF, ACT_NONE, EPI>(p, s); break;
    }
  }
}

}
}

#ifdef ASRX_WS_INSTANTIATE
#define ASRX_WS_EXTERN
#else
#define ASRX_WS_EXTERN extern
#endif
#define ASRX_WS_INST(ABF, EPI) \
  ASRX_WS_EXTERN template void asrx::wn::launch_ws_act<asrx::wn::ABF, asrx::wn::Epi::EPI>(const asrx::wn::Params&, hipStream_t);
#ifndef ASRX_WS_INSTANTIATE
ASRX_WS_INST(BF16A, Plain)
ASRX_WS_INST(F32A, Plain)
ASRX_WS_INST(F32A, Res)
ASRX_WS_INST(BF16A, Rot)
ASRX_WS_INST(F32A, Rot)
#endif
```

### asr-model_amd/csrc/rowops.hip

```cpp
#include "common.h"
#include <algorithm>
#include <mutex>
#include <map>
#include <unordered_map>
#include <utility>

namespace asrx {

constexpr int RW = 4;

__device__ __forceinline__ int64_t row_begin() { return (int64_t)blockIdx.x * RW + (threadIdx.x >> 6); }
__device__ __forceinline__ int64_t row_step() { return (int64_t)gridDim.x * RW; }

static unsigned row_grid(int64_t rows, int64_t cap = 8192) {
  int64_t g = (rows + RW - 1) / RW;
  if (g > cap) g = cap;
  if (g < 1) g = 1;
  return (unsigned)g;
}
static unsigned ew_grid(int64_t n, int64_t cap = 16384) {
  int64_t g = (n + 255) / 256;
  if (g > cap) g = cap;
  if (g < 1) g = 1;
  return (unsigned)g;
}

__device__ __forceinline__ void flush_partials(float* part, int n, float* dst) {
  __syncthreads();
  for (int j = threadIdx.x; j < n; j += 64 * RW) {
    float s = 0.f;
    for (int w = 0; w < RW; ++w) s += part[w * n + j];
    atomicAdd(dst + j, s);
  }
}

template <int E>
__device__ __forceinline__ int lane_feat(int lane, int e) {
  static_assert(E % 2 == 0, "row kernels take E = D / 64 even");
  return 128 * (e >> 1) + 2 * lane + (e & 1);
}
template <int E>
__device__ __forceinline__ void ld_lane(const float* __restrict__ src, int lane, float (&v)[E]) {
  const float2* s2 = reinterpret_cast<const float2*>(src);
#pragma unroll
  for (int e = 0; e < E / 2; ++e) {
    const float2 t = s2[64 * e + lane];
    v[2 * e] = t.x;
    v[2 * e + 1] = t.y;
  }
}
template <int E>
__device__ __forceinline__ void st_lane(float* __restrict__ dst, int lane, const float (&v)[E]) {
  float2* d2 = reinterpret_cast<float2*>(dst);
#pragma unroll
// ... 1464 lines not shown
    float s = 0.f;
    for (int k = 0; k < K; ++k) {
      const int64_t tt = t - k + pad;
      if (tt >= 0 && tt < T) s += w[c * K + k] * g[base + tt * C];
    }
    dx[i] = s;
  }
}

__global__ __launch_bounds__(256) void dwconv_bwd_w_kernel(const float* __restrict__ g, const float* __restrict__ x,
                                                           float* __restrict__ dw, float* __restrict__ db, int64_t B,
                                                           int64_t T, int C, int K, int64_t chunk) {
  __shared__ float red[4][64][17];
  const int c = blockIdx.x * 64 + (threadIdx.x & 63);
  const int part = threadIdx.x >> 6;
  const int64_t nch = (T + chunk - 1) / chunk;
  const int64_t b = blockIdx.y / nch;
  const int64_t t0 = (blockIdx.y % nch) * chunk;
  const int64_t t1 = min(T, t0 + chunk);
  const int pad = K / 2;
  float acc[16];
  float ab = 0.f;
#pragma unroll
  for (int k = 0; k < 16; ++k) acc[k] = 0.f;
  if (c < C) {
    for (int64_t t = t0 + part; t < t1; t += 4) {
      const float gv = g[(b * T + t) * C + c];
      ab += gv;
#pragma unroll
      for (int k = 0; k < 16; ++k) {
        if (k < K) {
          const int64_t tt = t + k - pad;
          if (tt >= 0 && tt < T) acc[k] += gv * x[(b * T + tt) * C + c];
        }
      }
    }
  }
  const int tl = threadIdx.x & 63;
#pragma unroll
  for (int k = 0; k < 16; ++k) red[part][tl][k] = acc[k];
  red[part][tl][16] = ab;
  __syncthreads();
  if (part == 0 && c < C) {
    for (int k = 0; k < K; ++k) {
      const float s = red[0][tl][k] + red[1][tl][k] + red[2][tl][k] + red[3][tl][k];
      atomicAdd(dw + c * K + k, s);
    }
    if (db) atomicAdd(db + c, red[0][tl][16] + red[1][tl][16] + red[2][tl][16] + red[3][tl][16]);
  }
}

constexpr int DW_R = 16;
enum { DW_PRE_NONE = 0, DW_PRE_GLU = 1, DW_PRE_GELU = 2 };

template <int K, bool FLIP, int PRE = DW_PRE_NONE>
__global__ __launch_bounds__(256) void dwconv_tile_kernel(const float4* __restrict__ x, const float* __restrict__ w,
                                                          const float* __restrict__ b, float4* __restrict__ y,
                                                          int B, int T, int C4, int ntile,
                                                          const float4* __restrict__ z) {
  constexpr int P = K / 2, W = DW_R + K - 1;
  static_assert(FLIP || PRE == DW_PRE_NONE, "PRE is an epilogue of the data-gradient form");
  const int64_t gid = (int64_t)blockIdx.x * 256 + threadIdx.x;
  if (gid >= (int64_t)B * ntile * C4) return;
  const int c4 = (int)(gid % C4);
  const int64_t rest = gid / C4;
  const int t0 = (int)(rest % ntile) * DW_R;
  const int64_t bb = rest / ntile;
  const float4* xs = x + bb * T * C4 + c4;
  float4 wk[K];
#pragma unroll
  for (int k = 0; k < K; ++k) {
    const int kk = FLIP ? K - 1 - k : k;
    const float* wc = w + (int64_t)(4 * c4) * K + kk;
    wk[k] = make_float4(wc[0], wc[K], wc[2 * K], wc[3 * K]);
  }
  float4 bias = make_float4(0.f, 0.f, 0.f, 0.f);
  if (b) bias = *reinterpret_cast<const float4*>(b + 4 * c4);
  float4 acc[DW_R];
#pragma unroll
  for (int r = 0; r < DW_R; ++r) acc[r] = bias;
#pragma unroll
  for (int j = 0; j < W; ++j) {
    const int row = t0 - P + j;
    float4 v = make_float4(0.f, 0.f, 0.f, 0.f);
    if (row >= 0 && row < T) v = xs[(int64_t)row * C4];
#pragma unroll
    for (int k = 0; k < K; ++k) {
      const int r = j - k;
      if (r >= 0 && r < DW_R) {
        acc[r].x += wk[k].x * v.x;
        acc[r].y += wk[k].y * v.y;
        acc[r].z += wk[k].z * v.z;
        acc[r].w += wk[k].w * v.w;
      }
    }
  }
  if constexpr (FLIP && PRE == DW_PRE_GLU) {
    const float4* zs = z + bb * T * 2 * C4 + c4;
    float4* ys = y + bb * T * 2 * C4 + c4;
#pragma unroll
    for (int r = 0; r < DW_R; ++r)
      if (t0 + r < T) {
        const int64_t o = (int64_t)(t0 + r) * 2 * C4;
        const float4 a = zs[o], q = zs[o + C4], g = acc[r];
        const float sx = sigmoid_f(q.x), sy = sigmoid_f(q.y), sz = sigmoid_f(q.z), sw = sigmoid_f(q.w);
        ys[o] = make_float4(g.x * sx, g.y * sy, g.z * sz, g.w * sw);
        ys[o + C4] = make_float4(g.x * a.x * sx * (1.f - sx), g.y * a.y * sy * (1.f - sy),
                                 g.z * a.z * sz * (1.f - sz), g.w * a.w * sw * (1.f - sw));
      }
  } else if constexpr (FLIP && PRE == DW_PRE_GELU) {
    const float4* zs = z + bb * T * C4 + c4;
    float4* ys = y + bb * T * C4 + c4;
#pragma unroll
    for (int r = 0; r < DW_R; ++r)
      if (t0 + r < T) {
        const float4 v = zs[(int64_t)(t0 + r) * C4], g = acc[r];
        ys[(int64_t)(t0 + r) * C4] =
            make_float4(g.x * gelu_grad(v.x), g.y * gelu_grad(v.y), g.z * gelu_grad(v.z), g.w * gelu_grad(v.w));
      }
  } else {
    float4* ys = y + bb * T * C4 + c4;
#pragma unroll
    for (int r = 0; r < DW_R; ++r)
      if (t0 + r < T) ys[(int64_t)(t0 + r) * C4] = acc[r];
  }
}

constexpr int DW_S = 4;

template <int K>
__global__ __launch_bounds__(256) void dwconv_wgrad_kernel(const float4* __restrict__ g, const float4* __restrict__ x,
                                                           float* __restrict__ dw, float* __restrict__ db, int T,
                                                           int C4, int nchunk) {
  constexpr int P = K / 2, W = DW_R + K - 1;
  __shared__ float4 red[4][32][K + 1];
  const int lane = threadIdx.x & 63, wid = threadIdx.x >> 6;
  const int cl = lane & 31, grp = wid * 2 + (lane >> 5);
  const int cchunks = (C4 + 31) / 32;
  const int cc = blockIdx.x % cchunks;
  const int chunk = (blockIdx.x / cchunks) % nchunk;
  const int64_t bb = blockIdx.x / ((int64_t)cchunks * nchunk);
  const int c4 = cc * 32 + cl;
  float4 acc[K + 1];
#pragma unroll
  for (int k = 0; k <= K; ++k) acc[k] = make_float4(0.f, 0.f, 0.f, 0.f);
  if (c4 < C4) {
    const float4* gs = g + bb * T * C4 + c4;
    const float4* xs = x + bb * T * C4 + c4;
    for (int s = 0; s < DW_S; ++s) {
      const int t0 = ((chunk * 8 + grp) * DW_S + s) * DW_R;
      if (t0 >= T) break;
      float4 gv[DW_R];
#pragma unroll
      for (int r = 0; r < DW_R; ++r) {
        gv[r] = (t0 + r < T) ? gs[(int64_t)(t0 + r) * C4] : make_float4(0.f, 0.f, 0.f, 0.f);
        acc[K].x += gv[r].x; acc[K].y += gv[r].y; acc[K].z += gv[r].z; acc[K].w += gv[r].w;
      }
#pragma unroll
      for (int j = 0; j < W; ++j) {
        const int row = t0 - P + j;
        float4 v = make_float4(0.f, 0.f, 0.f, 0.f);
        if (row >= 0 && row < T) v = xs[(int64_t)row * C4];
#pragma unroll
        for (int k = 0; k < K; ++k) {
          const int r = j - k;
          if (r >= 0 && r < DW_R) {
            acc[k].x += gv[r].x * v.x;
            acc[k].y += gv[r].y * v.y;
            acc[k].z += gv[r].z * v.z;
            acc[k].w += gv[r].w * v.w;
          }
        }
      }
    }
  }
#pragma unroll
  for (int k = 0; k <= K; ++k) {
    acc[k].x += __shfl_xor(acc[k].x, 32);
    acc[k].y += __shfl_xor(acc[k].y, 32);
    acc[k].z += __shfl_xor(acc[k].z, 32);
    acc[k].w += __shfl_xor(acc[k].w, 32);
    if (lane < 32) red[wid][cl][k] = acc[k];
  }
  __syncthreads();
  const int c_base = cc * 128;
  const int nch = min(128, 4 * C4 - c_base);
  const float* rf = reinterpret_cast<const float*>(&red[0][0][0]);
  constexpr int WS = 32 * (K + 1) * 4;
  for (int i = threadIdx.x; i < nch * K; i += 256) {
    const int c = i / K, k = i % K;
    const int off = ((c >> 2) * (K + 1) + k) * 4 + (c & 3);
    atomicAdd(dw + (int64_t)(c_base + c) * K + k, rf[off] + rf[WS + off] + rf[2 * WS + off] + rf[3 * WS + off]);
  }
  if (db)
    for (int c = threadIdx.x; c < nch; c += 256) {
      const int off = ((c >> 2) * (K + 1) + K) * 4 + (c & 3);
      atomicAdd(db + c_base + c, rf[off] + rf[WS + off] + rf[2 * WS + off] + rf[3 * WS + off]);
    }
}

template <int K>
static void dwconv_tiled(const float* x, const float* w, const float* b, float* y, const float* g, float* dx,
                         float* dw, float* db, int64_t B, int64_t T, int64_t C, hipStream_t stream) {
  const int C4 = (int)(C / 4);
  const int ntile = (int)((T + DW_R - 1) / DW_R);
  const int64_t threads = B * ntile * C4;
  const unsigned grid = (unsigned)((threads + 255) / 256);
  if (y) dwconv_tile_kernel<K, false><<<grid, 256, 0, stream>>>((const float4*)x, w, b, (float4*)y, (int)B, (int)T, C4,
                                                                 ntile, nullptr);
  if (dx) dwconv_tile_kernel<K, true><<<grid, 256, 0, stream>>>((const float4*)g, w, nullptr, (float4*)dx, (int)B,
                                                                 (int)T, C4, ntile, nullptr);
  if (dw) {
    const int nchunk = (int)((T + 8 * DW_S * DW_R - 1) / (8 * DW_S * DW_R));
    const int64_t blocks = B * nchunk * ((C4 + 31) / 32);
    dwconv_wgrad_kernel<K><<<(unsigned)blocks, 256, 0, stream>>>((const float4*)g, (const float4*)x, dw, db, (int)T,
                                                                   C4, nchunk);
  }
}

static bool dwconv_pre_ok(const float* g, const float* x, const float* z, const float* dz, int64_t B, int64_t T,
                          int64_t C, int64_t K, int pre) {
  const bool form = (pre == DW_PRE_GLU && K == 15) || (pre == DW_PRE_GELU && K == 3);
  const uintptr_t al = (uintptr_t)g | (uintptr_t)x | (uintptr_t)z | (uintptr_t)dz;
  return form && C % 4 == 0 && (al & 15) == 0 && B * T * C * (pre == DW_PRE_GLU ? 2 : 1) < (1LL << 31);
}

template <int K, int PRE>
static void dwconv_pre_bwd_launch(const float* g, const float* x, const float* z, const float* w, float* dz, float* dw,
                                  float* db, int64_t B, int64_t T, int64_t C, hipStream_t stream) {
  const int C4 = (int)(C / 4);
  const int ntile = (int)((T + DW_R - 1) / DW_R);
  const int64_t threads = B * ntile * C4;
  dwconv_tile_kernel<K, true, PRE><<<(unsigned)((threads + 255) / 256), 256, 0, stream>>>(
      (const float4*)g, w, nullptr, (float4*)dz, (int)B, (int)T, C4, ntile, (const float4*)z);
  if (dw) {
    const int nchunk = (int)((T + 8 * DW_S * DW_R - 1) / (8 * DW_S * DW_R));
    const int64_t blocks = B * nchunk * ((C4 + 31) / 32);
    dwconv_wgrad_kernel<K><<<(unsigned)blocks, 256, 0, stream>>>((const float4*)g, (const float4*)x, dw, db, (int)T,
                                                                   C4, nchunk);
  }
}

static bool dwconv_dispatch(const float* x, const float* w, const float* b, float* y, const float* g, float* dx,
                            float* dw, float* db, int64_t B, int64_t T, int64_t C, int64_t K, hipStream_t stream) {
  if (C % 4 != 0 || ((uintptr_t)(x ? x : g) & 15) || (y && ((uintptr_t)y & 15)) || (dx && ((uintptr_t)dx & 15)) ||
      (b && ((uintptr_t)b & 15)) || B * T * C >= (1LL << 31))
    return false;
  switch (K) {
    case 3: dwconv_tiled<3>(x, w, b, y, g, dx, dw, db, B, T, C, stream); return true;
    case 5: dwconv_tiled<5>(x, w, b, y, g, dx, dw, db, B, T, C, stream); return true;
    case 7: dwconv_tiled<7>(x, w, b, y, g, dx, dw, db, B, T, C, stream); return true;
    case 15: dwconv_tiled<15>(x, w, b, y, g, dx, dw, db, B, T, C, stream); return true;
    default: return false;
  }
}

__global__ __launch_bounds__(256) void bn_stats_kernel(const float* __restrict__ x, float* __restrict__ mean,
                                                       float* __restrict__ rstd, int64_t T, int C, float eps) {
  __shared__ float red[4][64];
  __shared__ float mu_s[64];
  const int b = blockIdx.y;
  const int tl = threadIdx.x & 63;
  const int c = blockIdx.x * 64 + tl;
  const int part = threadIdx.x >> 6;
  float s = 0.f;
  if (c < C)
    for (int64_t t = part; t < T; t += 4) s += x[((int64_t)b * T + t) * C + c];
  red[part][tl] = s;
  __syncthreads();
  if (part == 0) mu_s[tl] = (red[0][tl] + red[1][tl] + red[2][tl] + red[3][tl]) / T;
  __syncthreads();
  const float mu = mu_s[tl];
  float v = 0.f;
  if (c < C)
    for (int64_t t = part; t < T; t += 4) {
      const float d = x[((int64_t)b * T + t) * C + c] - mu;
      v += d * d;
    }
  __syncthreads();
  red[part][tl] = v;
  __syncthreads();
  if (part == 0 && c < C) {
    const float var = (red[0][tl] + red[1][tl] + red[2][tl] + red[3][tl]) / T;
    mean[(int64_t)b * C + c] = mu;
    rstd[(int64_t)b * C + c] = rsqrtf(var + eps);
  }
}
// ... 130 lines not shown
}

__global__ __launch_bounds__(256) void bn_bwd_stats_kernel(const float* __restrict__ g, const float* __restrict__ x,
                                                           const float* __restrict__ mean, const float* __restrict__ rstd,
                                                           const float* __restrict__ w, float* __restrict__ sg,
                                                           float* __restrict__ sgx, float* __restrict__ dw,
                                                           float* __restrict__ db, int64_t T, int C) {
  __shared__ float red[2][4][64];
  const int b = blockIdx.y;
  const int tl = threadIdx.x & 63;
  const int c = blockIdx.x * 64 + tl;
  const int part = threadIdx.x >> 6;
  float a = 0.f, ax = 0.f;
  if (c < C) {
    const float mu = mean[(int64_t)b * C + c], rs = rstd[(int64_t)b * C + c];
    for (int64_t t = part; t < T; t += 4) {
      const int64_t i = ((int64_t)b * T + t) * C + c;
      const float gv = g[i];
      a += gv;
      ax += gv * (x[i] - mu) * rs;
    }
  }
  red[0][part][tl] = a;
  red[1][part][tl] = ax;
  __syncthreads();
  if (part == 0 && c < C) {
    const float A = red[0][0][tl] + red[0][1][tl] + red[0][2][tl] + red[0][3][tl];
    const float AX = red[1][0][tl] + red[1][1][tl] + red[1][2][tl] + red[1][3][tl];
    sg[(int64_t)b * C + c] = A * w[c];
    sgx[(int64_t)b * C + c] = AX * w[c];
    atomicAdd(dw + c, AX);
    atomicAdd(db + c, A);
  }
}

__global__ void bn_bwd_apply_kernel(const float* __restrict__ g, const float* __restrict__ x,
                                    const float* __restrict__ mean, const float* __restrict__ rstd,
                                    const float* __restrict__ w, const float* __restrict__ sg,
                                    const float* __restrict__ sgx, float* __restrict__ dx, int64_t B, int64_t T, int C) {
  const int64_t total = B * T * C;
  for (int64_t i = (int64_t)blockIdx.x * blockDim.x + threadIdx.x; i < total; i += (int64_t)gridDim.x * blockDim.x) {
    const int64_t c = i % C;
    const int64_t b = i / (T * C);
    const int64_t s = b * C + c;
    const float rs = rstd[s];
    const float xh = (x[i] - mean[s]) * rs;
    dx[i] = rs * (g[i] * w[c] - sg[s] / T - xh * sgx[s] / T);
  }
}

__global__ void bn_silu_apply4_kernel(const float4* __restrict__ x, const float* __restrict__ mean,
                                      const float* __restrict__ rstd, const float* __restrict__ w,
                                      const float* __restrict__ bb, float4* __restrict__ y, uint32_t n4, uint32_t C4,
                                      uint32_t T, int per_sample) {
  for (uint32_t i = blockIdx.x * blockDim.x + threadIdx.x; i < n4; i += gridDim.x * blockDim.x) {
    const uint32_t row = i / C4, c0 = (i - row * C4) * 4u;
    const uint32_t s = per_sample ? (row / T) * (C4 * 4u) + c0 : c0;
    const float4 v = x[i];
    const float4 mu = *reinterpret_cast<const float4*>(mean + s), rs = *reinterpret_cast<const float4*>(rstd + s);
    const float4 wv = *reinterpret_cast<const float4*>(w + c0), bv = *reinterpret_cast<const float4*>(bb + c0);
    y[i] = make_float4(silu_f((v.x - mu.x) * rs.x * wv.x + bv.x), silu_f((v.y - mu.y) * rs.y * wv.y + bv.y),
                       silu_f((v.z - mu.z) * rs.z * wv.z + bv.z), silu_f((v.w - mu.w) * rs.w * wv.w + bv.w));
  }
}

__global__ void bn_silu_bwd_apply4_kernel(const float4* __restrict__ g, const float4* __restrict__ x,
                                          const float* __restrict__ mean, const float* __restrict__ rstd,
                                          const float* __restrict__ w, const float* __restrict__ bb,
                                          const float* __restrict__ sg, const float* __restrict__ sgx,
                                          float4* __restrict__ dx, uint32_t n4, uint32_t C4, uint32_t T) {
  const float Tf = (float)T;
  auto one = [&](float gv, float xv, float mu, float rs, float wc, float bc, float sgs, float sgxs)
                 __attribute__((always_inline)) {
    const float xh = (xv - mu) * rs;
    const float gz = gv * silu_grad(xh * wc + bc);
    return rs * (gz * wc - sgs / Tf - xh * sgxs / Tf);
  };
  for (uint32_t i = blockIdx.x * blockDim.x + threadIdx.x; i < n4; i += gridDim.x * blockDim.x) {
    const uint32_t row = i / C4, c0 = (i - row * C4) * 4u;
    const uint32_t s = (row / T) * (C4 * 4u) + c0;
    const float4 gv = g[i], xv = x[i];
    const float4 mu = *reinterpret_cast<const float4*>(mean + s), rs = *reinterpret_cast<const float4*>(rstd + s);
    const float4 wv = *reinterpret_cast<const float4*>(w + c0), bv = *reinterpret_cast<const float4*>(bb + c0);
    const float4 a = *reinterpret_cast<const float4*>(sg + s), ax = *reinterpret_cast<const float4*>(sgx + s);
    dx[i] = make_float4(one(gv.x, xv.x, mu.x, rs.x, wv.x, bv.x, a.x, ax.x),
                        one(gv.y, xv.y, mu.y, rs.y, wv.y, bv.y, a.y, ax.y),
                        one(gv.z, xv.z, mu.z, rs.z, wv.z, bv.z, a.z, ax.z),
                        one(gv.w, xv.w, mu.w, rs.w, wv.w, bv.w, a.w, ax.w));
  }
}

__global__ void stem1_fwd_kernel(const float* __restrict__ x, const float* __restrict__ W, const float* __restrict__ bias,
                                 float* __restrict__ y, int64_t B, int64_t T, int D) {
  const int64_t total = B * T * D;
  for (int64_t i = (int64_t)blockIdx.x * blockDim.x + threadIdx.x; i < total; i += (int64_t)gridDim.x * blockDim.x) {
    const int64_t o = i % D;
    const int64_t t = (i / D) % T;
    const int64_t b = i / (T * D);
    const float* xr = x + b * T;
    float s = bias[o];
    if (t > 0) s += W[o * 3 + 0] * xr[t - 1];
    s += W[o * 3 + 1] * xr[t];
    if (t + 1 < T) s += W[o * 3 + 2] * xr[t + 1];
    y[i] = s;
  }
}
__global__ __launch_bounds__(256) void stem1_bwd_w_kernel(const float* __restrict__ g, const float* __restrict__ x,
                                                          float* __restrict__ dW, float* __restrict__ db, int64_t B,
                                                          int64_t T, int D, int64_t chunk) {
  __shared__ float red[4][64][4];
  const int tl = threadIdx.x & 63;
  const int o = blockIdx.x * 64 + tl;
  const int part = threadIdx.x >> 6;
  const int64_t nch = (T + chunk - 1) / chunk;
  const int64_t b = blockIdx.y / nch;
// ... 805 lines not shown
                         int64_t sid_base, uint32_t key, float p, int act, int act2, hipStream_t stream) {
  const int64_t n = B * T * C;
  if (n == 0) return 0;
  ASRX_REQUIRE(act_dropout_vec_ok(z, y, res, n, C), "act_dropout: needs C %% 4 == 0 and 16-byte aligned tensors");
  LAUNCH_EW(act_dropout4_kernel<false>, n / 4, nullptr, reinterpret_cast<const float4*>(z),
            reinterpret_cast<const float4*>(res), reinterpret_cast<float4*>(y), (uint32_t)(n / 4), (uint32_t)(C / 4), (uint32_t)T, (uint32_t)C,
            (uint32_t)sid_base, key, p, act, act2);
  ASRX_LAUNCHED("asrx_act_dropout_fwd");
}

int asrx_act_dropout_bwd(const float* g, const float* z, float* dz, int64_t B, int64_t T, int64_t C,
                         int64_t sid_base, uint32_t key, float p, int act, int act2, hipStream_t stream) {
  const int64_t n = B * T * C;
  if (n == 0) return 0;
  ASRX_REQUIRE(act_dropout_vec_ok(g, z, dz, n, C), "act_dropout: needs C %% 4 == 0 and 16-byte aligned tensors");
  LAUNCH_EW(act_dropout4_kernel<true>, n / 4, reinterpret_cast<const float4*>(g), reinterpret_cast<const float4*>(z),
            nullptr, reinterpret_cast<float4*>(dz), (uint32_t)(n / 4), (uint32_t)(C / 4), (uint32_t)T, (uint32_t)C,
            (uint32_t)sid_base, key, p, act, act2);
  ASRX_LAUNCHED("asrx_act_dropout_bwd");
}

int asrx_dwconv_fwd(const float* x, const float* w, const float* b, float* y, int64_t B, int64_t T, int64_t C,
                    int64_t K, hipStream_t stream) {
  ASRX_REQUIRE(K % 2 == 1 && K <= 16, "dwconv: K must be odd and <= 15");
  if (B * T == 0) return 0;
  if (!dwconv_dispatch(x, w, b, y, nullptr, nullptr, nullptr, nullptr, B, T, C, K, stream))
    LAUNCH_EW(dwconv_fwd_kernel, B * T * C, x, w, b, y, B, T, (int)C, (int)K);
  ASRX_LAUNCHED("asrx_dwconv_fwd");
}

int asrx_dwconv_bwd(const float* g, const float* x, const float* w, float* dx, float* dw, float* db, int64_t B,
                    int64_t T, int64_t C, int64_t K, hipStream_t stream) {
  if (B * T == 0) return 0;
  if (dwconv_dispatch(x, w, nullptr, nullptr, g, dx, dw, db, B, T, C, K, stream)) ASRX_LAUNCHED("asrx_dwconv_bwd");
  if (dx) LAUNCH_EW(dwconv_bwd_data_kernel, B * T * C, g, w, dx, B, T, (int)C, (int)K);
  const int64_t chunk = 256;
  const int64_t nch = (T + chunk - 1) / chunk;
  dim3 grid((unsigned)((C + 63) / 64), (unsigned)(B * nch));
  dwconv_bwd_w_kernel<<<grid, 256, 0, stream>>>(g, x, dw, db, B, T, (int)C, (int)K, chunk);
  ASRX_LAUNCHED("asrx_dwconv_bwd");
}

int asrx_dwconv_pre_bwd(const float* g, const float* x, const float* z, const float* w, float* dz, float* dw,
                        float* db, int64_t B, int64_t T, int64_t C, int64_t K, int pre, hipStream_t stream) {
  if (B * T == 0) return 0;
  ASRX_REQUIRE(dwconv_pre_ok(g, x, z, dz, B, T, C, K, pre),
               "asrx_dwconv_pre_bwd: GLU -> k15 or GELU -> k3 with C %% 4 == 0, 16-byte aligned tensors and "
               "fewer than 2^31 elements");
  if (pre == DW_PRE_GLU) dwconv_pre_bwd_launch<15, DW_PRE_GLU>(g, x, z, w, dz, dw, db, B, T, C, stream);
  else dwconv_pre_bwd_launch<3, DW_PRE_GELU>(g, x, z, w, dz, dw, db, B, T, C, stream);
  ASRX_LAUNCHED("asrx_dwconv_pre_bwd");
}

int asrx_bn_fwd(const float* x, const float* w, const float* b, float* y, float* mean, float* rstd, int64_t B,
                int64_t T, int64_t C, float eps, int use_batch_stats, hipStream_t stream) {
  if (B * T == 0) return 0;
  if (use_batch_stats) {
    if (C % 4 == 0 && ((uintptr_t)x & 15) == 0) {
      const int C4 = (int)(C / 4);
      bn_stats4_kernel<<<(unsigned)(B * ((C4 + 31) / 32)), 1024, 0, stream>>>((const float4*)x, mean, rstd, (int)T,
                                                                             C4, eps);
    } else {
      dim3 grid((unsigned)((C + 63) / 64), (unsigned)B);
      bn_stats_kernel<<<grid, 256, 0, stream>>>(x, mean, rstd, T, (int)C, eps);
    }
  }
  LAUNCH_EW(bn_apply_kernel, B * T * C, x, mean, rstd, w, b, y, B, T, (int)C, use_batch_stats);
  ASRX_LAUNCHED("asrx_bn_fwd");
}

int asrx_bn_bwd(const float* g, const float* x, const float* mean, const float* rstd, const float* w, float* sg_ws,
                float* sgx_ws, float* dx, float* dw, float* db, int64_t B, int64_t T, int64_t C, hipStream_t stream) {
  if (B * T == 0) return 0;
  if (C % 4 == 0 && ((uintptr_t)x & 15) == 0 && ((uintptr_t)g & 15) == 0 && ((uintptr_t)mean & 15) == 0 &&
      ((uintptr_t)rstd & 15) == 0) {
    const int C4 = (int)(C / 4);
    bn_bwd_stats4_kernel<false><<<(unsigned)(B * ((C4 + 31) / 32)), 1024, 0, stream>>>(
        (const float4*)g, (const float4*)x, mean, rstd, w, sg_ws, sgx_ws, dw, db, (int)T, C4, nullptr);
  } else {
    dim3 grid((unsigned)((C + 63) / 64), (unsigned)B);
    bn_bwd_stats_kernel<<<grid, 256, 0, stream>>>(g, x, mean, rstd, w, sg_ws, sgx_ws, dw, db, T, (int)C);
  }
  LAUNCH_EW(bn_bwd_apply_kernel, B * T * C, g, x, mean, rstd, w, sg_ws, sgx_ws, dx, B, T, (int)C);
  ASRX_LAUNCHED("asrx_bn_bwd");
}

static bool bn_silu_vec_ok(std::initializer_list<const void*> ps, int64_t B, int64_t T, int64_t C) {
  uintptr_t al = 0;
  for (const void* p : ps) al |= (uintptr_t)p;
  return C % 4 == 0 && (al & 15) == 0 && B * T * C < (1LL << 31);
}

int asrx_bn_silu_fwd(const float* x, const float* w, const float* b, float* y, float* mean, float* rstd, int64_t B,
                     int64_t T, int64_t C, float eps, int use_batch_stats, hipStream_t stream) {
  if (B * T == 0) return 0;
  ASRX_REQUIRE(bn_silu_vec_ok({x, w, b, y, mean, rstd}, B, T, C),
               "asrx_bn_silu_fwd: needs C %% 4 == 0, 16-byte aligned tensors and B*T*C < 2^31");
  const int C4 = (int)(C / 4);
  if (use_batch_stats)
    bn_stats4_kernel<<<(unsigned)(B * ((C4 + 31) / 32)), 1024, 0, stream>>>((const float4*)x, mean, rstd, (int)T, C4,
                                                                           eps);
  const int64_t n4 = B * T * C4;
  LAUNCH_EW(bn_silu_apply4_kernel, n4, (const float4*)x, mean, rstd, w, b, (float4*)y, (uint32_t)n4, (uint32_t)C4,
            (uint32_t)T, use_batch_stats);
  ASRX_LAUNCHED("asrx_bn_silu_fwd");
}

int asrx_bn_silu_bwd(const float* g, const float* x, const float* mean, const float* rstd, const float* w,
                     const float* b, float* sg_ws, float* sgx_ws, float* dx, float* dw, float* db, int64_t B,
                     int64_t T, int64_t C, hipStream_t stream) {
  if (B * T == 0) return 0;
  ASRX_REQUIRE(bn_silu_vec_ok({g, x, mean, rstd, w, b, sg_ws, sgx_ws, dx}, B, T, C),
               "asrx_bn_silu_bwd: needs C %% 4 == 0, 16-byte aligned tensors and B*T*C < 2^31");
  const int C4 = (int)(C / 4);
  bn_bwd_stats4_kernel<true><<<(unsigned)(B * ((C4 + 31) / 32)), 1024, 0, stream>>>(
      (const float4*)g, (const float4*)x, mean, rstd, w, sg_ws, sgx_ws, dw, db, (int)T, C4, b);
  const int64_t n4 = B * T * C4;
  LAUNCH_EW(bn_silu_bwd_apply4_kernel, n4, (const float4*)g, (const float4*)x, mean, rstd, w, b, sg_ws, sgx_ws,
            (float4*)dx, (uint32_t)n4, (uint32_t)C4, (uint32_t)T);
  ASRX_LAUNCHED("asrx_bn_silu_bwd");
}

int asrx_stem1_fwd(const float* x, const float* W, const float* bias, float* y, int64_t B, int64_t T, int64_t D,
                   hipStream_t stream) {
  if (B * T == 0) return 0;
  LAUNCH_EW(stem1_fwd_kernel, B * T * D, x, W, bias, y, B, T, (int)D);
  ASRX_LAUNCHED("asrx_stem1_fwd");
}

int asrx_stem1_bwd(const float* g, const float* x, float* dW, float* db, int64_t B, int64_t T, int64_t D,
                   hipStream_t stream) {
  if (B * T == 0) return 0;
  const int64_t chunk = 256, nch = (T + chunk - 1) / chunk;
  dim3 grid((unsigned)((D + 63) / 64), (unsigned)(B * nch));
  stem1_bwd_w_kernel<<<grid, 256, 0, stream>>>(g, x, dW, db, B, T, (int)D, chunk);
  ASRX_LAUNCHED("asrx_stem1_bwd");
}

int asrx_embed_fwd(const int64_t* ids, const float* E, float* y, int64_t rows, int64_t d, hipStream_t stream) {
  if (rows == 0) return 0;
  LAUNCH_EW(embed_fwd_kernel, rows * d, ids, E, y, rows, (int)d);
  ASRX_LAUNCHED("asrx_embed_fwd");
}

int asrx_embed_bwd(const int64_t* ids, const float* g, float* dE, int64_t rows, int64_t d, hipStream_t stream) {
  if (rows == 0) return 0;
  LAUNCH_EW(embed_bwd_kernel, rows * d, ids, g, dE, rows, (int)d);
  ASRX_LAUNCHED("asrx_embed_bwd");
}

int asrx_ce_fwd(const float* z, const int64_t* labels, float* loss, float* lse, int64_t rows, int64_t V,
                hipStream_t stream) {
  if (rows == 0) return 0;
  ASRX_REQUIRE(rows < (1LL << 31), "ce: too many rows");
  ce_fwd_kernel<<<(unsigned)rows, 256, 0, stream>>>(z, labels, loss, lse, V);
  ASRX_LAUNCHED("asrx_ce_fwd");
}

int asrx_ce_bwd(const float* z, const int64_t* labels, const float* lse, const float* scale, float* dz, int64_t rows,
                int64_t V, hipStream_t stream) {
  if (rows == 0) return 0;
  ce_bwd_kernel<<<(unsigned)rows, 256, 0, stream>>>(z, labels, lse, scale, dz, V);
  ASRX_LAUNCHED("asrx_ce_bwd");
}

}

namespace asrx {
__global__ void policy_noise_kernel(float* out, int64_t B, int64_t layers, int64_t sid_base, uint32_t key) {
  const int64_t n = B * layers * 3;
  for (int64_t j = (int64_t)blockIdx.x * blockDim.x + threadIdx.x; j < n; j += (int64_t)gridDim.x * blockDim.x) {
    const int64_t k = j % 3, i = (j / 3) % layers, b = j / (3 * layers);
    out[j] = noise_gumbel(key, (uint32_t)(((sid_base + b) * 64 + i) * 3 + k));
  }
}
}
extern "C" int asrx_policy_noise(float* out, int64_t B, int64_t layers, int64_t sid_base, uint32_t key,
                                 hipStream_t stream) {
  ASRX_REQUIRE(layers <= 64, "policy noise: at most 64 layers");
  if (B * layers == 0) return 0;
  asrx::policy_noise_kernel<<<(unsigned)((B * layers * 3 + 255) / 256), 256, 0, stream>>>(out, B, layers, sid_base, key);
  ASRX_LAUNCHED("asrx_policy_noise");
}

ASRX_NOISE_EPOCH_SETTER(asrx_set_noise_epoch_rowops)
```

### include/asrx.h

```cpp
#ifndef ASRX_H
#define ASRX_H
#include <stdint.h>

#ifdef __cplusplus
extern "C" {
#endif

typedef void* asrx_stream_t;

const char* asrx_last_error(void);
int asrx_abi_version(void);
uint32_t asrx_noise_hash(uint32_t key, uint32_t idx);
int asrx_set_noise_epoch(uint32_t epoch, asrx_stream_t stream);
int asrx_set_gemm_variant(int variant);
int asrx_set_attn_variant(int variant);
int asrx_set_wgrad_variant(int variant);

int asrx_mel_frames(int64_t n_samples);
int64_t asrx_logmel_ws_bytes(int64_t B, int64_t N);
int asrx_logmel(const float* wav, int64_t B, int64_t N, int64_t ld_wav, const float* consts,
                const float* fbw, const int* fbs, float* out, int layout, int64_t ld_out,
                void* ws, float* pool, int64_t T_pool, asrx_stream_t stream);
int asrx_wave_pool(const float* wav, int64_t B, int64_t N, int64_t ld_wav, int64_t T, float* out,
                   asrx_stream_t stream);
// ... 288 lines not shown
  const unsigned short *m2_wb;
  const float *m2_b;
  int64_t H1;
  int32_t a1_bf16, n_layers;
  const asrx_msheath_layer* layers;
} asrx_msheath_plan;
int64_t asrx_msheath_plan_bytes(void);
int64_t asrx_msheath_layer_bytes(void);
int64_t asrx_msheath_fwd_ws_bytes(const asrx_msheath_plan* plan, int64_t B, int64_t L, int64_t D);
int asrx_msheath_fwd(const asrx_msheath_plan* plan, const float* x0, const float* gpol, int64_t ld_gpol, float* y,
                     void* ws, int64_t ws_bytes, int64_t B, int64_t L, int64_t D, asrx_stream_t stream);
int asrx_axpy_row2(const float* x, const float* s1, const float* s2, const float* y, float* out, int64_t rows,
                   int64_t d, asrx_stream_t stream);
int asrx_axpy_row2_bwd(const float* g, const float* s1, const float* s2, const float* y, float* dy, float* ds1,
                       float* ds2, int64_t rows, int64_t d, asrx_stream_t stream);
int asrx_jump_axpy_inplace(const float* xin, float* xout, const float* s1, const float* s2, const float* y,
                           const float* orig, const float* act, const float* alpha, const float* beta, const float* gam,
                           int64_t B, int64_t L, int64_t d, asrx_stream_t stream);
int asrx_jump_select4(const float* xn, const float* orig, const float* xold, const float* act, const float* alpha,
                      const float* beta, const float* gam, float* out, int64_t B, int64_t L, int64_t d,
                      asrx_stream_t stream);
int asrx_jump_select4_bwd(const float* g, const float* xn, const float* orig, const float* act, const float* alpha,
                          const float* beta, float* dxn, float* dorig, float* dxold, float* dalpha, float* dbeta,
                          float* dgam, int64_t B, int64_t L, int64_t d, asrx_stream_t stream);
int asrx_seg_colsum(const float* x, float* out, int64_t B, int64_t L, int64_t d, float scale, int accumulate,
                    asrx_stream_t stream);
int asrx_colsum(const float* x, float* out, int64_t rows, int64_t d, asrx_stream_t stream);
int asrx_seg_colsum_det(const float* x, float* part, float* out, int64_t B, int64_t L, int64_t d, float scale,
                        asrx_stream_t stream);
int asrx_colsum_ld(const float* x, int64_t ld, float* out, int64_t rows, int64_t d, asrx_stream_t stream);
int asrx_add_rows(const float* x, const float* t, const float* u, float* out, int64_t B, int64_t L, int64_t d,
                  asrx_stream_t stream);
int asrx_lincomb(const float* x, const float* y, const float* z, float a, float b, float c, float* out, int64_t n,
                 asrx_stream_t stream);
int asrx_policy_noise(float* out, int64_t B, int64_t layers, int64_t sid_base, uint32_t key,
                      asrx_stream_t stream);

int asrx_act_fwd(const float* x, float* y, int64_t n, int act, asrx_stream_t stream);
int asrx_act_bwd(const float* g, const float* x, float* dx, int64_t n, int act, asrx_stream_t stream);
int asrx_glu_fwd(const float* x, float* y, int64_t rows, int64_t C, asrx_stream_t stream);
int asrx_glu_bwd(const float* g, const float* x, float* dx, int64_t rows, int64_t C, asrx_stream_t stream);
int asrx_dropout(const float* x, float* y, int64_t B, int64_t T, int64_t C, int64_t sid_base, uint32_t key,
                 float p, asrx_stream_t stream);
int asrx_act_dropout_fwd(const float* z, const float* res, float* y, int64_t B, int64_t T, int64_t C,
                         int64_t sid_base, uint32_t key, float p, int act, int act2, asrx_stream_t stream);
int asrx_act_dropout_bwd(const float* g, const float* z, float* dz, int64_t B, int64_t T, int64_t C,
                         int64_t sid_base, uint32_t key, float p, int act, int act2, asrx_stream_t stream);
int asrx_dwconv_fwd(const float* x, const float* w, const float* b, float* y, int64_t B, int64_t T, int64_t C,
                    int64_t K, asrx_stream_t stream);
int asrx_dwconv_bwd(const float* g, const float* x, const float* w, float* dx, float* dw, float* db, int64_t B,
                    int64_t T, int64_t C, int64_t K, asrx_stream_t stream);
int asrx_dwconv_pre_bwd(const float* g, const float* x, const float* z, const float* w, float* dz, float* dw,
                        float* db, int64_t B, int64_t T, int64_t C, int64_t K, int pre, asrx_stream_t stream);
int asrx_bn_fwd(const float* x, const float* w, const float* b, float* y, float* mean, float* rstd, int64_t B,
                int64_t T, int64_t C, float eps, int use_batch_stats, asrx_stream_t stream);
int asrx_bn_bwd(const float* g, const float* x, const float* mean, const float* rstd, const float* w, float* sg_ws,
                float* sgx_ws, float* dx, float* dw, float* db, int64_t B, int64_t T, int64_t C,
                asrx_stream_t stream);
int asrx_bn_silu_fwd(const float* x, const float* w, const float* b, float* y, float* mean, float* rstd, int64_t B,
                     int64_t T, int64_t C, float eps, int use_batch_stats, asrx_stream_t stream);
int asrx_bn_silu_bwd(const float* g, const float* x, const float* mean, const float* rstd, const float* w,
                     const float* b, float* sg_ws, float* sgx_ws, float* dx, float* dw, float* db, int64_t B,
                     int64_t T, int64_t C, asrx_stream_t stream);
int asrx_stem1_fwd(const float* x, const float* W, const float* bias, float* y, int64_t B, int64_t T, int64_t D,
                   asrx_stream_t stream);
int asrx_stem1_bwd(const float* g, const float* x, float* dW, float* db, int64_t B, int64_t T, int64_t D,
                   asrx_stream_t stream);

int asrx_embed_fwd(const int64_t* ids, const float* E, float* y, int64_t rows, int64_t d, asrx_stream_t stream);
int asrx_embed_bwd(const int64_t* ids, const float* g, float* dE, int64_t rows, int64_t d, asrx_stream_t stream);
int asrx_ce_fwd(const float* z, const int64_t* labels, float* loss, float* lse, int64_t rows, int64_t V,
                asrx_stream_t stream);
int asrx_ce_bwd(const float* z, const int64_t* labels, const float* lse, const float* scale, float* dz,
                int64_t rows, int64_t V, asrx_stream_t stream);

int asrx_maxfactor_param_bytes(void);
int asrx_maxfactor_step(const void* table, int np, int64_t nrows, int64_t ncols, int64_t ncc, int64_t nmats,
                        int64_t nitems, float* ws, asrx_stream_t stream);
int asrx_maxfactor_step_ex(const void* table, int np, int64_t nrows, int64_t ncols, int64_t ncc, int64_t nmats,
                           int64_t nitems, float* ws, const float* ctl, int clip_any, asrx_stream_t stream);

int asrx_grad_stats_param_bytes(void);
int asrx_grad_stats(const void* table, int np, int64_t nitems, float inv_scale, float max_norm, float eps,
                    float* stats, float* ws, asrx_stream_t stream);


int asrx_ce_fwd1(const float* z, const int64_t* labels, float* loss_r, float* lse, float* loss, float* count,
                 int64_t rows, int64_t V, asrx_stream_t stream);
int asrx_ce_bwd2(const float* z, const int64_t* labels, const float* lse, const float* g, const float* count, float* dz,
                 int64_t rows, int64_t V, asrx_stream_t stream);
int asrx_gemm_wn_ce(const void* A, int64_t lda, const unsigned short* W, int64_t ldw, unsigned short* Zb, int64_t ldc,
                    float* part, int64_t M, int64_t N, int64_t K, int nj, asrx_stream_t stream);
int asrx_ce_part_fwd(const float* part, int64_t nparts, const unsigned short* zb, const int64_t* labels, float* loss_r,
                     float* lse, float* loss, float* count, int64_t rows, int64_t V, asrx_stream_t stream);
int asrx_ce_bwd_bf16(const unsigned short* zb, const int64_t* labels, const float* lse, const float* g,
                     const float* count, unsigned short* dzb, int64_t rows, int64_t V, asrx_stream_t stream);
int asrx_gemm_wn_ce_f32(const void* A, int64_t lda, const unsigned short* W, int64_t ldw, float* Zf, int64_t ldc,
                        float* part, int64_t M, int64_t N, int64_t K, int nj, asrx_stream_t stream);
int asrx_ce_part_fwd_f32(const float* part, int64_t nparts, const float* zf, const int64_t* labels, float* loss_r,
                         float* lse, float* loss, float* count, int64_t rows, int64_t V, asrx_stream_t stream);
int asrx_ce_bwd_f32in(const float* zf, const int64_t* labels, const float* lse, const float* g, const float* count,
                      unsigned short* dzb, int64_t rows, int64_t V, asrx_stream_t stream);
int asrx_gemm_wn_head(const void* A, int64_t lda, const unsigned short* W, int64_t ldw, float* part,
                      const int64_t* labels, float* zlab, int64_t M, int64_t N, int64_t K, int nj,
                      asrx_stream_t stream);
int asrx_head_merge(const float* part, int64_t nparts, const float* zlab, const int64_t* labels, int64_t* pred,
                    float* loss_r, float* lse, float* loss, float* count, int64_t* correct, int64_t rows, int64_t V,
                    asrx_stream_t stream);
int asrx_gemm_wn_gact(const void* A, int a_bf16, int64_t lda, const unsigned short* W, int64_t ldw, const float* bias,
                      const float* G, int64_t ldg, unsigned short* gz, int64_t ldc, float* db, int64_t M, int64_t N,
                      int64_t K, int act, int nj, asrx_stream_t stream);
int asrx_gemm_wn_rot(const void* A, int a_bf16, int64_t lda, const unsigned short* W, int64_t ldw, float* C, float* Z,
                     int64_t ldc, const float* bias, const float* m, const float* tab, int64_t L, int64_t hd,
                     float scale, int64_t M, int64_t N, int64_t K, int nj, asrx_stream_t stream);
int asrx_gemm_lt(const void* A, int64_t lda, const unsigned short* W, int64_t ldw, void* C, int c_bf16, int64_t ldc,
                 const float* bias, int64_t M, int64_t N, int64_t K, float alpha, float beta, asrx_stream_t stream);
int asrx_gemm_wn_res(const float* A, int64_t lda, const unsigned short* W, int64_t ldw, float* C, int64_t ldc,
                     const float* bias, const float* R, int64_t ldr, int64_t M, int64_t N, int64_t K, int nj,
                     asrx_stream_t stream);
int asrx_act_bwd_bias(const float* g, const float* z, unsigned short* gz, float* db, int64_t rows, int64_t N, int act,
                      asrx_stream_t stream);
int asrx_wgrad_bf16_ab(const void* A, int64_t lda, const void* B, int b_bf16, int64_t ldb, float* C, int64_t ldc,
                       int64_t M, int64_t N, int64_t R, int64_t splitk, asrx_stream_t stream);
int asrx_wgrad_bias(const void* A, int a_bf16, int64_t lda, const void* B, int b_bf16, int64_t ldb, float* C,
                    int64_t ldc, float* db, int64_t M, int64_t N, int64_t R, int64_t splitk, asrx_stream_t stream);
int asrx_wgrad_split(const float* A, int64_t lda, const void* B, int b_bf16, int64_t ldb, float* C, int64_t ldc,
                     float* C2, int64_t ldc2, int64_t msplit, int64_t M, int64_t N, int64_t R, int64_t splitk,
                     asrx_stream_t stream);
int asrx_bn_running(const float* mean, const float* rstd, float* rm, float* rv, int64_t* nbt, int64_t B, int64_t C,
                    int64_t T, float eps, float momentum, asrx_stream_t stream);
int asrx_rsqrt_eps(const float* v, float* out, int64_t n, float eps, asrx_stream_t stream);
int asrx_conv3_weight(const float* g, const float* v, int64_t Co, int64_t Ci, float* Wt, unsigned short* Wtb, float* Wf,
                      unsigned short* Wfb, float* nrm, asrx_stream_t stream);
int asrx_conv3_weight_bwd(const float* dWt, const float* g, const float* v, const float* nrm, int64_t Co, int64_t Ci,
                          float* dg, float* dv, asrx_stream_t stream);
int asrx_blend_fwd(const float* d, const float* g, const float* blend, float* out, int64_t n, asrx_stream_t stream);
int asrx_blend_bwd(const float* go, const float* d, const float* g, const float* blend, float* dd, float* dg,
                   float* dblend, int64_t n, asrx_stream_t stream);
int asrx_add_segments(const float* src, int64_t n, float* d0, float* d1, float* d2, int64_t nseg, asrx_stream_t stream);
int asrx_cat3(const float* a, const float* b, const float* c, int64_t n, float* out, asrx_stream_t stream);


int asrx_pitch_dio(const float* x, int64_t ldx, int64_t B, int64_t N, double fs, double f0_floor, double f0_ceil,
                   double fp, double allowed_range, const double* lc, int64_t c, const double* nut,
                   const int64_t* nut_off, const int64_t* nut_len, const double* bf0, int64_t nb, double* mean,
                   double* hp, double* f, double* ev, int64_t cap, double* cand, double* score, double* work,
                   double* f0, int64_t F, asrx_stream_t stream);
int asrx_pitch_stonemask(const float* x, int64_t ldx, int64_t B, int64_t N, double fs, const double* f0, double fp,
                         int64_t F, double* out, asrx_stream_t stream);

#ifdef __cplusplus
}
#endif
#endif
```

Measured before the change: 5622 audio-sec/sec.

## Fuse conformer conv-module tail: BN-SiLU bf16 output, GEMM with dropout+residual epilogue

In the encoder conv module's training path, batch-norm+SiLU now writes bf16 directly, and the point2 projection runs as a wide GEMM whose epilogue applies dropout and adds the residual. This removes a separate dropout_add pass and an fp32 round trip of the activation. In backward, the next layer's dwconv-pre backward kernel also emits the dropout-masked gradient and hands it over through a DropHand object, so the separate dropout-backward kernel is skipped when the hand-off matches. This adds kernel instantiations and version-checked state passed between autograd nodes, and the bf16 activation loses some precision.

```diff
diff --git a/asr-model_amd/asrx/gemm.py b/asr-model_amd/asrx/gemm.py
--- a/asr-model_amd/asrx/gemm.py
+++ b/asr-model_amd/asrx/gemm.py
@@ -313,6 +313,30 @@
     lib.call("asrx_gemm_wn_rot", lib.ptr(x2), ab, K, lib.ptr(Wb), Wb.stride(0), lib.ptr(y), lib.ptr(preact), N,
              lib.ptr(b), lib.ptr(m), lib.ptr(tab), L, hd, float(scale), M, N, K, nj, lib.stream())
     probe.end("gemm", e0, 2.0 * M * N * K, ("wn", M, N, K, nj, 0, "rot", preact is not None, False, ab, 0, -1))
+    return y
+
+
+def dropres_ok(x, W, res) -> bool:
+    if x.dim() != 3 or not is_bf16(x) or not x.is_cuda or not x.is_contiguous() or not res.is_contiguous():
+        return False
+    N, K = W.shape[0], W.numel() // W.shape[0]
+    M = x.shape[0] * x.shape[1]
+    return (use_wide(K) and x.shape[2] == K and N % 4 == 0 and M > 0 and res.dtype == torch.float32
+            and tuple(res.shape) == (x.shape[0], x.shape[1], N) and x.data_ptr() % 16 == 0
+            and res.data_ptr() % 16 == 0 and M * max(N, K) < 1 << 31 and _nj(M, N) in (1, 3))
+
+
+def linear_dropout_res_fwd(x, W, b, res, sid_base, key, p):
+    B, T, K = x.shape
+    M, N = B * T, W.shape[0]
+    Wb = weight_bf16(W.view(N, -1))
+    y = torch.empty(B, T, N, device=x.device)
+    nj = _nj(M, N)
+    lib.require_gpu(x, Wb, y, res)
+    e0 = probe.begin("gemm")
+    lib.call("asrx_gemm_dropres", lib.ptr(x), 1, K, lib.ptr(Wb), Wb.stride(0), lib.ptr(y), N, lib.ptr(b), lib.ptr(res), N,
+             T, sid_base, key & 0xFFFFFFFF, float(p), M, N, K, nj, lib.stream())
+    probe.end("gemm", e0, 2.0 * M * N * K, ("wn", M, N, K, nj, 0, "dropres", False, True, 1, 0, -1))
     return y
 
 
diff --git a/asr-model_amd/asrx/lib.py b/asr-model_amd/asrx/lib.py
--- a/asr-model_amd/asrx/lib.py
+++ b/asr-model_amd/asrx/lib.py
@@ -141,6 +141,11 @@
     "asrx_dwconv_pre_bwd": (_i32, [_p, _p, _p, _p, _p, _p, _p, _i64, _i64, _i64, _i64, _i32, _p]),
     "asrx_bn_silu_fwd": (_i32, [_p, _p, _p, _p, _p, _p, _i64, _i64, _i64, _f32, _i32, _p]),
     "asrx_bn_silu_bwd": (_i32, [_p, _p, _p, _p, _p, _p, _p, _p, _p, _p, _p, _i64, _i64, _i64, _p]),
+    "asrx_bn_silu_fwd_bf16": (_i32, [_p, _p, _p, _p, _p, _p, _i64, _i64, _i64, _f32, _i32, _p]),
+    "asrx_dwconv_pre_bwd_drop": (_i32, [_p, _p, _p, _p, _p, _p, _p, _p, _i64, _i64, _i64, _i64, _i32, _i64, _u32,
+                                        _f32, _p]),
+    "asrx_gemm_dropres": (_i32, [_p, _i32, _i64, _p, _i64, _p, _i64, _p, _p, _i64, _i64, _i64, _u32, _f32, _i64, _i64,
+                                 _i64, _i32, _p]),
     "asrx_stem1_fwd": (_i32, [_p, _p, _p, _p, _i64, _i64, _i64, _p]),
     "asrx_stem1_bwd": (_i32, [_p, _p, _p, _p, _i64, _i64, _i64, _p]),
     "asrx_embed_fwd": (_i32, [_p, _p, _p, _i64, _i64, _p]),
diff --git a/asr-model_amd/asrx/model.py b/asr-model_amd/asrx/model.py
--- a/asr-model_amd/asrx/model.py
+++ b/asr-model_amd/asrx/model.py
@@ -106,14 +106,13 @@
         y = ops.glu_dwconv(y, self.depth.weight, self.depth.bias)
         if self.training:
             stats = []
-            y = ops.batch_norm_silu(y, self.bn.weight, self.bn.bias, self.bn.eps, stats)
+            y = ops.batch_norm_silu(y, self.bn.weight, self.bn.bias, self.bn.eps, stats, gemm_only=True)
             self._update_running(stats[0], y.shape[1])
-        else:
-            y = ops.batch_norm_silu_eval(y, self.bn.weight, self.bn.bias, self.bn.running_mean,
-                                         self.bn.running_var, self.bn.eps)
+            return ops.linear_dropout_add(res, y, self.point2.weight, self.point2.bias, sid_base,
+                                          noise.key(site + ".cl"), 0.1)
+        y = ops.batch_norm_silu_eval(y, self.bn.weight, self.bn.bias, self.bn.running_mean,
+                                     self.bn.running_var, self.bn.eps)
         y = ops.linear(y, self.point2.weight, self.point2.bias)
-        if self.training:
-            return ops.dropout_add(res, y, sid_base, noise.key(site + ".cl"), 0.1)
         return ops.add(res, y)
 
     @torch.no_grad()
diff --git a/asr-model_amd/asrx/ops.py b/asr-model_amd/asrx/ops.py
--- a/asr-model_amd/asrx/ops.py
+++ b/asr-model_amd/asrx/ops.py
@@ -337,6 +337,68 @@
             and x.dtype == torch.float32 and r.shape[-1] == N and x.is_cuda and G._nj(M, N) in (1, 3)):
         return LinearRes.apply(r, x, W, b, sink_of(x))
     return add(r, linear(x, W, b))
+
+
+class LinearDropRes(torch.autograd.Function):
+
+    @staticmethod
+    def forward(ctx, res, x, W, b, sid_base, key, p, sink, hand):
+        x, res = _c(x), _c(res)
+        ctx.sink, ctx.hand = sink, hand
+        ctx.set_materialize_grads(False)
+        out = G.linear_dropout_res_fwd(x, W, b, res, sid_base, key, p)
+        ctx.args = (sid_base, key, p)
+        ctx.dW, ctx.db = _direct(ctx, 2, W), _direct(ctx, 3, b)
+        ctx.has_b = b is not None
+        ctx.save_for_backward(x, W, b if ctx.db else None)
+        return out
+
+    @staticmethod
+    def backward(ctx, g):
+        x, W3, b = ctx.saved_tensors
+        if g is None:
+            return (None,) * 9
+        g = _f32(g)
+        sid_base, key, p = ctx.args
+        W = W3.view(W3.shape[0], -1)
+        B, T, N = g.shape
+        hand, ctx.hand = ctx.hand, None
+        dy = hand.take(g) if hand is not None else None
+        if dy is None:
+            dy = _E(g.shape, device=g.device)
+            lib.call("asrx_dropout", _P(g), _P(dy), B, T, N, sid_base, key & 0xFFFFFFFF, float(p), _S())
+        dx = None
+        if ctx.needs_input_grad[1]:
+            if ctx.sink is not None:
+                buf, acc = ctx.sink.target(x)
+                G.linear_dgrad(dy, W, out=buf, beta=float(acc))
+            else:
+                dx = G.linear_dgrad(dy, W)
+        dW = db = None
+        gb = None
+        if ctx.has_b and ctx.needs_input_grad[3]:
+            gb = _gbuf(b, True) if ctx.db else torch.zeros(N, device=g.device)
+        if ctx.needs_input_grad[2]:
+            gW = _gbuf(W3, ctx.dW)
+            G.linear_wgrad(dy, x, out=gW.view(W.shape), accumulate=True, db=gb)
+            dW = _gret(W3, gW, ctx.dW)
+        elif gb is not None:
+            colsum(dy, out=gb)
+        if gb is not None:
+            db = _gret(b, gb, ctx.db)
+        return g if ctx.needs_input_grad[0] else None, dx, dW, db, None, None, None, None, None
+
+
+def linear_dropout_add(res, x, W, b, sid_base, key, p):
+    res = _c(res)
+    if enc_tail_fused() and G.dropres_ok(x, W, res) and (b is None or b.data_ptr() % 16 == 0):
+        _noise_rows_ok(sid_base + x.shape[0], W.shape[0], x.shape[1])
+        hand = DropHand(sid_base, key, p, res.shape) if _grad_needed(res, x, W, b) else None
+        out = LinearDropRes.apply(res, x, W, b, sid_base, key, p, sink_of(x), hand)
+        if hand is not None and out.requires_grad:
+            out._asrx_drop_hand = hand
+        return out
+    return dropout_add(res, linear(x, W, b), sid_base, key, p)
 
 
 class KVProjFn(torch.autograd.Function):
@@ -1451,6 +1513,35 @@
 FUSED_ENCODER = True
 DW_PRE = {"glu": 1, "gelu": 2}
 _DW_PRE_K = {"glu": 15, "gelu": 3}
+ENC_TAIL_FUSED = __import__("os").environ.get("ASRX_ENC_TAIL_FUSED", "1") != "0"
+
+
+def enc_tail_fused() -> bool:
+    return ENC_TAIL_FUSED and FUSED_ENCODER and prec.get() == prec.PREC_BF16 and torch.is_grad_enabled()
+
+
+class DropHand:
+    __slots__ = ("sid_base", "key", "p", "shape", "src", "dy", "version")
+
+    def __init__(self, sid_base, key, p, shape):
+        self.sid_base, self.key, self.p, self.shape = sid_base, key, p, tuple(shape)
+        self.src = self.dy = self.version = None
+
+    def give(self, src, dy):
+        self.src, self.dy, self.version = src, dy, src._version
+
+    def take(self, g):
+        src, dy, ver = self.src, self.dy, self.version
+        self.src = self.dy = self.version = None
+        if (src is None or g.data_ptr() != src.data_ptr() or g.shape != src.shape or g.dtype != src.dtype
+                or not g.is_contiguous() or g._version != ver):
+            HAND_STATS["missed"] += 1
+            return None
+        HAND_STATS["taken"] += 1
+        return dy
+
+
+HAND_STATS = {"taken": 0, "missed": 0}
 
 
 def _aligned(t):
@@ -1461,8 +1552,9 @@
 class PreDWConv(torch.autograd.Function):
 
     @staticmethod
-    def forward(ctx, z, w, b, pre):
+    def forward(ctx, z, w, b, pre, hand=None):
         z = _c(z)
+        ctx.hand = hand
         B, T = z.shape[:2]
         C, K = w.shape[0], w.shape[-1]
         if z.dim() != 3 or z.shape[-1] != (2 * C if pre == "glu" else C):
@@ -1487,9 +1579,19 @@
         K = w.shape[-1]
         dz = _E(z.shape, device=z.device)
         dw, db = _gbuf(w, ctx.dw), _gbuf(b, ctx.db)
-        lib.call("asrx_dwconv_pre_bwd", _P(g), _P(x), _P(z), _P(w), _P(dz), _P(dw), _P(db), B, T, C, K,
-                 DW_PRE[ctx.pre], _S())
-        return dz, _gret(w, dw, ctx.dw), _gret(b, db, ctx.db), None
+        hand, ctx.hand = ctx.hand, None
+        if hand is not None and ctx.pre == "gelu" and hand.shape == tuple(z.shape):
+            dzd = _E(z.shape, device=z.device)
+            lib.call("asrx_dwconv_pre_bwd_drop", _P(g), _P(x), _P(z), _P(w), _P(dz), _P(dzd), _P(dw), _P(db), B, T, C, K,
+                     DW_PRE[ctx.pre], hand.sid_base, hand.key & 0xFFFFFFFF, float(hand.p), _S())
+            hand.give(dz, dzd)
+        else:
+            lib.call("asrx_dwconv_pre_bwd", _P(g), _P(x), _P(z), _P(w), _P(dz), _P(dw), _P(db), B, T, C, K,
+                     DW_PRE[ctx.pre], _S())
+        return dz, _gret(w, dw, ctx.dw), _gret(b, db, ctx.db), None, None
+
+
+ENC_TAIL_DROP_HAND = True
 
 
 def _pre_dwconv(z, w, pre):
@@ -1506,22 +1608,26 @@
 
 
 def act_dwconv(x, name, w, b):
+    hand = getattr(x, "_asrx_drop_hand", None)
     x = _c(x)
     if name == "gelu" and _pre_dwconv(x, w, "gelu"):
-        return PreDWConv.apply(x, w, b, "gelu")
+        return PreDWConv.apply(x, w, b, "gelu", hand if (ENC_TAIL_DROP_HAND and enc_tail_fused()) else None)
     return DWConv.apply(act(x, name), w, b)
 
 
 class BatchNormSiLU(torch.autograd.Function):
 
     @staticmethod
-    def forward(ctx, x, w, b, eps, stats):
+    def forward(ctx, x, w, b, eps, stats, out_bf16=False, osink=None):
         x = _c(x)
         B, T, C = x.shape
+        ctx.osink = osink
+        ctx.set_materialize_grads(False)
         mean = _E(B, C, device=x.device)
         rstd = _E(B, C, device=x.device)
-        y = _E(x.shape, device=x.device)
-        lib.call("asrx_bn_silu_fwd", _P(x), _P(w), _P(b), _P(y), _P(mean), _P(rstd), B, T, C, float(eps), 1, _S())
+        y = _E(x.shape, device=x.device, dtype=torch.bfloat16 if out_bf16 else torch.float32)
+        lib.call("asrx_bn_silu_fwd_bf16" if out_bf16 else "asrx_bn_silu_fwd", _P(x), _P(w), _P(b), _P(y), _P(mean),
+                 _P(rstd), B, T, C, float(eps), 1, _S())
         if stats is not None:
             stats.append((mean, rstd))
         ctx.dw, ctx.db = _direct(ctx, 1, w), _direct(ctx, 2, b)
@@ -1531,6 +1637,10 @@
     @staticmethod
     def backward(ctx, g):
         x, w, mean, rstd, b = ctx.saved_tensors
+        osink, ctx.osink = ctx.osink, None
+        g = grad_in(g, osink)
+        if g is None:
+            return None, None, None, None, None, None, None
         g = _aligned(g)
         B, T, C = x.shape
         sg = _E(B, C, device=x.device)
@@ -1539,7 +1649,7 @@
         dw, db = _gbuf(w, ctx.dw), _gbuf(b, ctx.db)
         lib.call("asrx_bn_silu_bwd", _P(g), _P(x), _P(mean), _P(rstd), _P(w), _P(b), _P(sg), _P(sgx), _P(dx), _P(dw),
                  _P(db), B, T, C, _S())
-        return dx, _gret(w, dw, ctx.dw), _gret(b, db, ctx.db), None, None
+        return dx, _gret(w, dw, ctx.dw), _gret(b, db, ctx.db), None, None, None, None
 
 
 def _bn_silu_ok(x, *ps):
@@ -1547,10 +1657,12 @@
             and all(t.data_ptr() % 16 == 0 for t in (x,) + ps))
 
 
-def batch_norm_silu(x, w, b, eps, stats):
+def batch_norm_silu(x, w, b, eps, stats, gemm_only=False):
     x = _c(x)
     if _bn_silu_ok(x, w, b):
-        return BatchNormSiLU.apply(x, w, b, eps, stats)
+        ob = bool(gemm_only and enc_tail_fused() and prec.bf16_storage() and G.use_wide(x.shape[-1]))
+        osink = new_sink(ob) if _grad_needed(x, w, b) else None
+        return out_sink(BatchNormSiLU.apply(x, w, b, eps, stats, ob, osink), osink)
     return act(BatchNormPS.apply(x, w, b, eps, stats), "silu")
 
 
diff --git a/asr-model_amd/csrc/common.h b/asr-model_amd/csrc/common.h
--- a/asr-model_amd/csrc/common.h
+++ b/asr-model_amd/csrc/common.h
@@ -254,6 +254,11 @@
   if (ep != 0u) key ^= mix32(ep * 0x9E3779B9U + 0x7F4A7C15U);
   return key;
 }
+__device__ __forceinline__ uint32_t noise_key_at(uint32_t key, const uint32_t* ep_addr) {
+  const uint32_t ep = *(const __attribute__((address_space(4))) uint32_t*)ep_addr;
+  if (ep != 0u) key ^= mix32(ep * 0x9E3779B9U + 0x7F4A7C15U);
+  return key;
+}
 __device__ __forceinline__ float noise_uniform_k(uint32_t key, uint32_t idx) {
   uint32_t h = mix32(mix32(idx ^ key) + (key * 0x9E3779B9U + 0x632BE5ABU));
   return ((float)(h >> 9) + 0.5f) * (1.0f / 8388608.0f);
diff --git a/asr-model_amd/csrc/gemm_p2.h b/asr-model_amd/csrc/gemm_p2.h
--- a/asr-model_amd/csrc/gemm_p2.h
+++ b/asr-model_amd/csrc/gemm_p2.h
@@ -113,13 +113,15 @@
 #endif
 
 constexpr bool p2_built(int nj, bool abf, Epi e) {
-  return e == Epi::Plain ? nj == 2 || nj == 3 : e == Epi::Res ? nj == 3 && !abf : e == Epi::Rot && nj == 3;
+  return e == Epi::Plain ? nj == 2 || nj == 3
+         : e == Epi::Res ? nj == 3 && !abf
+         : e == Epi::DropRes ? nj == 3 && abf : e == Epi::Rot && nj == 3;
 }
 
 template <int NJ, bool ABF, int ACT, Epi EPI>
 __global__ __launch_bounds__(p2::NT2, 2) void gemm_p2_kernel(Params p, int ntiles) {
   static_assert(p2_built(NJ, ABF, EPI), "not a gemm_p2_kernel instantiation (p2_built)");
-  static_assert(EPI == Epi::Plain || ACT == ACT_NONE, "the residual and rotary epilogues take no activation");
+  static_assert(EPI == Epi::Plain || ACT == ACT_NONE, "the residual, dropout and rotary epilogues take no activation");
   using namespace p2;
   typedef Geo<NJ, ABF> GE;
   constexpr int BN = GE::BN, NT = 2 * NJ;
@@ -310,4 +312,5 @@
 ASRX_P2_INST(2, F32A, Plain)
 ASRX_P2_INST(2, BF16A, Plain)
 ASRX_P2_INST(3, F32A, Res)
-#endif
+ASRX_P2_INST(3, BF16A, DropRes)
+#endif
diff --git a/asr-model_amd/csrc/gemm_p2_dropres.hip b/asr-model_amd/csrc/gemm_p2_dropres.hip
--- /dev/null
+++ b/asr-model_amd/csrc/gemm_p2_dropres.hip
@@ -0,0 +1,4 @@
+#define ASRX_P2_INSTANTIATE
+#include "gemm_p2.h"
+
+ASRX_P2_INST(3, BF16A, DropRes)
diff --git a/asr-model_amd/csrc/gemm_wn.hip b/asr-model_amd/csrc/gemm_wn.hip
--- a/asr-model_amd/csrc/gemm_wn.hip
+++ b/asr-model_amd/csrc/gemm_wn.hip
@@ -253,6 +253,35 @@
   p.Rres = R;
   p.ldr = (int)ldr;
   return launched(run_wide<wn::Epi::Res>(p, 0, nj, 0, stream), "asrx_gemm_wn_res");
+}
+
+extern "C" const uint32_t* asrx_noise_epoch_addr_rowops(void);
+
+extern "C" int asrx_gemm_dropres(const void* A, int a_bf16, int64_t lda, const unsigned short* W, int64_t ldw, float* C,
+                                 int64_t ldc, const float* bias, const float* R, int64_t ldr, int64_t T,
+                                 int64_t sid_base, uint32_t key, float p, int64_t M, int64_t N, int64_t K, int nj,
+                                 hipStream_t stream) {
+  const bool rows = T > 0 && T <= 8192 && M % T == 0 && sid_base >= 0 && p >= 0.f && p < 1.f;
+  if (int rc = wide_check("asrx_gemm_dropres", A, a_bf16, lda, W, ldw, M, N, K,
+                          {((uintptr_t)C & 15) == 0 && ((uintptr_t)R & 15) == 0, "A/W/C/R must be 16-byte aligned"},
+                          {N % 4 == 0 && ldc % 4 == 0 && ldr % 4 == 0, "K, ldw % 8; lda % 4 (8 bf16); N, ldc, ldr % 4"},
+                          T > 0 ? nullptr : "empty problem",
+                          rows ? nullptr : "T in 1..8192 dividing M, sid_base >= 0, p in [0, 1)"))
+    return rc;
+  ASRX_REQUIRE((sid_base + M / T) * N * 8192 <= (1LL << 32), "asrx_gemm_dropres: the noise index overflows 32 bits");
+  ASRX_REQUIRE(R && R != C, "asrx_gemm_dropres: a residual input distinct from C is required");
+  ASRX_REQUIRE(nj == 1 || nj == 3, "asrx_gemm_dropres: nj 1 or 3");
+  ASRX_REQUIRE(a_bf16, "asrx_gemm_dropres: bf16-stored A only (no fp32-A instance is built)");
+  wn::Params q = wide_params(A, lda, W, ldw, C, ldc, bias, nullptr, M, N, K);
+  q.Rres = R;
+  q.ldr = (int)ldr;
+  q.dr_T = (int)T;
+  q.dr_sid = (uint32_t)sid_base;
+  q.dr_key = key;
+  q.dr_p = p;
+  q.dr_epoch = asrx_noise_epoch_addr_rowops();
+  ASRX_REQUIRE(q.dr_epoch, "asrx_gemm_dropres: no noise epoch address");
+  return launched(run_wide<wn::Epi::DropRes>(q, 0, nj, a_bf16, stream), "asrx_gemm_dropres");
 }
 
 extern "C" int asrx_gemm_wn_rot(const void* A, int a_bf16, int64_t lda, const unsigned short* W, int64_t ldw,
diff --git a/asr-model_amd/csrc/gemm_wr.h b/asr-model_amd/csrc/gemm_wr.h
--- a/asr-model_amd/csrc/gemm_wr.h
+++ b/asr-model_amd/csrc/gemm_wr.h
@@ -16,6 +16,7 @@
   CE,
   Head,
   Res,
+  DropRes,
   GAct,
   Rot
 };
@@ -44,6 +45,10 @@
   int ce_ld;
   const float* Rres;
   int ldr;
+  int dr_T;
+  uint32_t dr_sid, dr_key;
+  float dr_p;
+  const uint32_t* dr_epoch;
   const float* G;
   int ldg;
   float* dB;
@@ -162,16 +167,35 @@
                      mm * (x.z * t.w + x.w * t.z));
 }
 
+__device__ __forceinline__ float4 dropres_apply(const Params& p, float4 x, int row, int col, uint32_t key, float sc) {
+#pragma clang fp contract(off)
+  const uint32_t T = (uint32_t)p.dr_T, b = (uint32_t)row / T, t = (uint32_t)row - b * T;
+  const uint32_t base = ((p.dr_sid + b) * (uint32_t)p.N + (uint32_t)col) * 8192u + t;
+  const float4 o = *reinterpret_cast<const float4*>(p.Rres + (int64_t)row * p.ldr + col);
+  const float d0 = noise_uniform_k(key, base) >= p.dr_p ? x.x * sc : 0.f;
+  const float d1 = noise_uniform_k(key, base + 8192u) >= p.dr_p ? x.y * sc : 0.f;
+  const float d2 = noise_uniform_k(key, base + 2u * 8192u) >= p.dr_p ? x.z * sc : 0.f;
+  const float d3 = noise_uniform_k(key, base + 3u * 8192u) >= p.dr_p ? x.w * sc : 0.f;
+  return make_float4(o.x + d0, o.y + d1, o.z + d2, o.w + d3);
+}
+
 template <int NJ, int ACT, Epi EPI = Epi::Plain>
 __device__ __forceinline__ void epilogue_lds(const Params& p, f32x4 (&acc)[4][2 * NJ], const float* bsl, int m0,
                                              int n0, int wm, int wn, int lr, int lk, float* ep) {
-  constexpr bool RES = EPI == Epi::Res, ROT = EPI == Epi::Rot;
-  static_assert(EPI == Epi::Plain || ((RES || ROT) && ACT == ACT_NONE), "plain, or residual / rotary without activation");
+  constexpr bool RES = EPI == Epi::Res, ROT = EPI == Epi::Rot, DROP = EPI == Epi::DropRes;
+  static_assert(EPI == Epi::Plain || ((RES || ROT || DROP) && ACT == ACT_NONE),
+                "plain, or residual / dropout-residual / rotary without activation");
   constexpr int NT = 2 * NJ, W = EpLds<NJ>::W, LD = EpLds<NJ>::LD, W4 = W / 4;
   constexpr int PER = 16 * W4 / 64;
   static_assert((16 * W4) % 64 == 0, "slice must split evenly over the wave");
   const int lane = threadIdx.x & 63;
   const int cbase = n0 + wn * W;
+  uint32_t dkey = 0u;
+  float dsc = 0.f;
+  if constexpr (DROP) {
+    dkey = noise_key_at(p.dr_key, p.dr_epoch);
+    dsc = 1.0f / (1.0f - p.dr_p);
+  }
 #pragma unroll
   for (int mt = 0; mt < 4; ++mt) {
 #pragma unroll
@@ -215,6 +239,7 @@
         __builtin_nontemporal_store(f32x4{x.x, x.y, x.z, x.w},
                                     reinterpret_cast<f32x4*>(p.Z + (int64_t)row * p.ldc + col));
       if constexpr (ROT) x = rot_apply(p, x, row, col);
+      if constexpr (DROP) x = dropres_apply(p, x, row, col, dkey, dsc);
       __builtin_nontemporal_store(f32x4{act_t<ACT>(x.x), act_t<ACT>(x.y), act_t<ACT>(x.z), act_t<ACT>(x.w)},
                                   reinterpret_cast<f32x4*>(dst));
     }
@@ -755,6 +780,7 @@
     case Epi::CE: return !conv && abf;
     case Epi::Head: return !conv && abf;
     case Epi::Res: return !conv && !abf && nj != 2;
+    case Epi::DropRes: return !conv && abf && nj != 2;
     case Epi::GAct: return !conv && nj == 3;
     case Epi::Rot: return !conv && nj != 2;
   }
@@ -764,7 +790,7 @@
 template <int NJ, bool CONV, bool ABF, Epi EPI>
 __global__ __launch_bounds__(NTHR, 1) void gemm_wr_kernel(Params p, int ntiles) {
   constexpr bool RT = EPI == Epi::Router, HEAD = EPI == Epi::Head, CE = EPI == Epi::CE || HEAD;
-  constexpr bool RES = EPI == Epi::Res, GA = EPI == Epi::GAct, ROT = EPI == Epi::Rot;
+  constexpr bool RES = EPI == Epi::Res, GA = EPI == Epi::GAct, ROT = EPI == Epi::Rot, DROP = EPI == Epi::DropRes;
   static_assert(!HEAD || (CE && ABF), "the head epilogue is a variant of the bf16-A CE instantiation");
   static_assert(wr_built(NJ, CONV, ABF, EPI), "not a gemm_wr_kernel instantiation (wr_built)");
   typedef Cfg<NJ> CF;
@@ -953,6 +979,8 @@
         epilogue_lds<NJ, ACT_NONE, Epi::Res>(p, acc, bsl, m0, n0, wm, wn, lr, lk, ep);
       } else if constexpr (ROT) {
         epilogue_lds<NJ, ACT_NONE, Epi::Rot>(p, acc, bsl, m0, n0, wm, wn, lr, lk, ep);
+      } else if constexpr (DROP) {
+        epilogue_lds<NJ, ACT_NONE, Epi::DropRes>(p, acc, bsl, m0, n0, wm, wn, lr, lk, ep);
       } else if constexpr (GA) {
         switch (p.act) {
           case ACT_GELU: epilogue_gact<NJ, ACT_GELU>(p, acc, bsl, m0, n0, wm, wn, lr, lk, ep); break;
@@ -1040,6 +1068,8 @@
 ASRX_WR_INST(3, ROWS, BF16A, CE)
 ASRX_WR_INST(1, ROWS, F32A, Res)
 ASRX_WR_INST(3, ROWS, F32A, Res)
+ASRX_WR_INST(1, ROWS, BF16A, DropRes)
+ASRX_WR_INST(3, ROWS, BF16A, DropRes)
 ASRX_WR_INST(3, ROWS, F32A, GAct)
 ASRX_WR_INST(3, ROWS, BF16A, GAct)
 ASRX_WR_INST(1, ROWS, BF16A, Rot)
diff --git a/asr-model_amd/csrc/gemm_wr_dropres.hip b/asr-model_amd/csrc/gemm_wr_dropres.hip
--- /dev/null
+++ b/asr-model_amd/csrc/gemm_wr_dropres.hip
@@ -0,0 +1,5 @@
+#define ASRX_WR_INSTANTIATE
+#include "gemm_wr.h"
+
+ASRX_WR_INST(1, ROWS, BF16A, DropRes)
+ASRX_WR_INST(3, ROWS, BF16A, DropRes)
diff --git a/asr-model_amd/csrc/gemm_ws.h b/asr-model_amd/csrc/gemm_ws.h
--- a/asr-model_amd/csrc/gemm_ws.h
+++ b/asr-model_amd/csrc/gemm_ws.h
@@ -54,7 +54,9 @@
 
 }
 
-constexpr bool ws_built(bool abf, Epi e) { return e == Epi::Plain || e == Epi::Rot || (e == Epi::Res && !abf); }
+constexpr bool ws_built(bool abf, Epi e) {
+  return e == Epi::Plain || e == Epi::Rot || (e == Epi::Res && !abf) || (e == Epi::DropRes && abf);
+}
 
 template <bool ABF, int ACT, Epi EPI>
 __global__ __launch_bounds__(ws::WTHR, 1) void gemm_ws_kernel(Params p, int nS, int lanes) {
@@ -325,6 +327,7 @@
 ASRX_WS_INST(BF16A, Plain)
 ASRX_WS_INST(F32A, Plain)
 ASRX_WS_INST(F32A, Res)
+ASRX_WS_INST(BF16A, DropRes)
 ASRX_WS_INST(BF16A, Rot)
 ASRX_WS_INST(F32A, Rot)
 #endif
diff --git a/asr-model_amd/csrc/gemm_ws_dropres.hip b/asr-model_amd/csrc/gemm_ws_dropres.hip
--- /dev/null
+++ b/asr-model_amd/csrc/gemm_ws_dropres.hip
@@ -0,0 +1,4 @@
+#define ASRX_WS_INSTANTIATE
+#include "gemm_ws.h"
+
+ASRX_WS_INST(BF16A, DropRes)
diff --git a/asr-model_amd/csrc/rowops.hip b/asr-model_amd/csrc/rowops.hip
--- a/asr-model_amd/csrc/rowops.hip
+++ b/asr-model_amd/csrc/rowops.hip
@@ -1,5 +1,6 @@
 #include "common.h"
 #include <algorithm>
+#include <atomic>
 #include <mutex>
 #include <map>
 #include <unordered_map>
@@ -1570,14 +1571,27 @@
 
 constexpr int DW_R = 16;
 enum { DW_PRE_NONE = 0, DW_PRE_GLU = 1, DW_PRE_GELU = 2 };
-
-template <int K, bool FLIP, int PRE = DW_PRE_NONE>
+struct DwDrop {
+  float4* out;
+  uint32_t sid_base, key;
+  float p;
+};
+
+__device__ __forceinline__ float4 dw_drop_value(float4 v, uint32_t key, uint32_t base, float p, float sc) {
+  float r[4] = {v.x, v.y, v.z, v.w};
+#pragma unroll
+  for (int j = 0; j < 4; ++j) r[j] = noise_uniform_k(key, base + (uint32_t)j * 8192u) >= p ? r[j] * sc : 0.f;
+  return make_float4(r[0], r[1], r[2], r[3]);
+}
+
+template <int K, bool FLIP, int PRE = DW_PRE_NONE, bool DROP = false>
 __global__ __launch_bounds__(256) void dwconv_tile_kernel(const float4* __restrict__ x, const float* __restrict__ w,
                                                           const float* __restrict__ b, float4* __restrict__ y,
                                                           int B, int T, int C4, int ntile,
-                                                          const float4* __restrict__ z) {
+                                                          const float4* __restrict__ z, DwDrop drop) {
   constexpr int P = K / 2, W = DW_R + K - 1;
   static_assert(FLIP || PRE == DW_PRE_NONE, "PRE is an epilogue of the data-gradient form");
+  static_assert(!DROP || PRE == DW_PRE_GELU, "DROP: the dropout of the GELU data gradient");
   const int64_t gid = (int64_t)blockIdx.x * 256 + threadIdx.x;
   if (gid >= (int64_t)B * ntile * C4) return;
   const int c4 = (int)(gid % C4);
@@ -1629,12 +1643,18 @@
   } else if constexpr (FLIP && PRE == DW_PRE_GELU) {
     const float4* zs = z + bb * T * C4 + c4;
     float4* ys = y + bb * T * C4 + c4;
+    float4* os = DROP ? drop.out + bb * T * C4 + c4 : nullptr;
+    const uint32_t key = DROP ? noise_key(drop.key) : 0u;
+    const float sc = DROP ? 1.0f / (1.0f - drop.p) : 0.f;
+    const uint32_t base0 = ((drop.sid_base + (uint32_t)bb) * (4u * (uint32_t)C4) + 4u * (uint32_t)c4) * 8192u;
 #pragma unroll
     for (int r = 0; r < DW_R; ++r)
       if (t0 + r < T) {
         const float4 v = zs[(int64_t)(t0 + r) * C4], g = acc[r];
-        ys[(int64_t)(t0 + r) * C4] =
+        const float4 d =
             make_float4(g.x * gelu_grad(v.x), g.y * gelu_grad(v.y), g.z * gelu_grad(v.z), g.w * gelu_grad(v.w));
+        ys[(int64_t)(t0 + r) * C4] = d;
+        if constexpr (DROP) os[(int64_t)(t0 + r) * C4] = dw_drop_value(d, key, base0 + (uint32_t)(t0 + r), drop.p, sc);
       }
   } else {
     float4* ys = y + bb * T * C4 + c4;
@@ -1725,9 +1745,9 @@
   const int64_t threads = B * ntile * C4;
   const unsigned grid = (unsigned)((threads + 255) / 256);
   if (y) dwconv_tile_kernel<K, false><<<grid, 256, 0, stream>>>((const float4*)x, w, b, (float4*)y, (int)B, (int)T, C4,
-                                                                 ntile, nullptr);
+                                                                 ntile, nullptr, DwDrop{});
   if (dx) dwconv_tile_kernel<K, true><<<grid, 256, 0, stream>>>((const float4*)g, w, nullptr, (float4*)dx, (int)B,
-                                                                 (int)T, C4, ntile, nullptr);
+                                                                 (int)T, C4, ntile, nullptr, DwDrop{});
   if (dw) {
     const int nchunk = (int)((T + 8 * DW_S * DW_R - 1) / (8 * DW_S * DW_R));
     const int64_t blocks = B * nchunk * ((C4 + 31) / 32);
@@ -1743,14 +1763,15 @@
   return form && C % 4 == 0 && (al & 15) == 0 && B * T * C * (pre == DW_PRE_GLU ? 2 : 1) < (1LL << 31);
 }
 
-template <int K, int PRE>
+template <int K, int PRE, bool DROP = false>
 static void dwconv_pre_bwd_launch(const float* g, const float* x, const float* z, const float* w, float* dz, float* dw,
-                                  float* db, int64_t B, int64_t T, int64_t C, hipStream_t stream) {
+                                  float* db, int64_t B, int64_t T, int64_t C, hipStream_t stream,
+                                  DwDrop drop = DwDrop{}) {
   const int C4 = (int)(C / 4);
   const int ntile = (int)((T + DW_R - 1) / DW_R);
   const int64_t threads = B * ntile * C4;
-  dwconv_tile_kernel<K, true, PRE><<<(unsigned)((threads + 255) / 256), 256, 0, stream>>>(
-      (const float4*)g, w, nullptr, (float4*)dz, (int)B, (int)T, C4, ntile, (const float4*)z);
+  dwconv_tile_kernel<K, true, PRE, DROP><<<(unsigned)((threads + 255) / 256), 256, 0, stream>>>(
+      (const float4*)g, w, nullptr, (float4*)dz, (int)B, (int)T, C4, ntile, (const float4*)z, drop);
   if (dw) {
     const int nchunk = (int)((T + 8 * DW_S * DW_R - 1) / (8 * DW_S * DW_R));
     const int64_t blocks = B * nchunk * ((C4 + 31) / 32);
@@ -1987,15 +2008,22 @@
 __global__ void bn_silu_apply4_kernel(const float4* __restrict__ x, const float* __restrict__ mean,
                                       const float* __restrict__ rstd, const float* __restrict__ w,
                                       const float* __restrict__ bb, float4* __restrict__ y, uint32_t n4, uint32_t C4,
-                                      uint32_t T, int per_sample) {
+                                      uint32_t T, int per_sample, uint2* __restrict__ yb) {
   for (uint32_t i = blockIdx.x * blockDim.x + threadIdx.x; i < n4; i += gridDim.x * blockDim.x) {
     const uint32_t row = i / C4, c0 = (i - row * C4) * 4u;
     const uint32_t s = per_sample ? (row / T) * (C4 * 4u) + c0 : c0;
     const float4 v = x[i];
     const float4 mu = *reinterpret_cast<const float4*>(mean + s), rs = *reinterpret_cast<const float4*>(rstd + s);
     const float4 wv = *reinterpret_cast<const float4*>(w + c0), bv = *reinterpret_cast<const float4*>(bb + c0);
-    y[i] = make_float4(silu_f((v.x - mu.x) * rs.x * wv.x + bv.x), silu_f((v.y - mu.y) * rs.y * wv.y + bv.y),
-                       silu_f((v.z - mu.z) * rs.z * wv.z + bv.z), silu_f((v.w - mu.w) * rs.w * wv.w + bv.w));
+    const float4 o = make_float4(silu_f((v.x - mu.x) * rs.x * wv.x + bv.x), silu_f((v.y - mu.y) * rs.y * wv.y + bv.y),
+                                 silu_f((v.z - mu.z) * rs.z * wv.z + bv.z), silu_f((v.w - mu.w) * rs.w * wv.w + bv.w));
+    if (yb) {
+      typedef __attribute__((ext_vector_type(4))) __bf16 bf16x4;
+      const bf16x4 h = {(__bf16)o.x, (__bf16)o.y, (__bf16)o.z, (__bf16)o.w};
+      yb[i] = __builtin_bit_cast(uint2, h);
+    } else {
+      y[i] = o;
+    }
   }
 }
 
@@ -2907,6 +2935,20 @@
   ASRX_LAUNCHED("asrx_dwconv_pre_bwd");
 }
 
+int asrx_dwconv_pre_bwd_drop(const float* g, const float* x, const float* z, const float* w, float* dz, float* dzd,
+                             float* dw, float* db, int64_t B, int64_t T, int64_t C, int64_t K, int pre,
+                             int64_t sid_base, uint32_t key, float p, hipStream_t stream) {
+  if (B * T == 0) return 0;
+  ASRX_REQUIRE(pre == DW_PRE_GELU && dzd && ((uintptr_t)dzd & 15) == 0 && dwconv_pre_ok(g, x, z, dz, B, T, C, K, pre),
+               "asrx_dwconv_pre_bwd_drop: GELU -> k3 with C %% 4 == 0, 16-byte aligned tensors and fewer than 2^31 "
+               "elements");
+  ASRX_REQUIRE(T <= 8192 && sid_base >= 0 && (sid_base + B) * C * 8192 <= (1LL << 32) && p >= 0.f && p < 1.f,
+               "asrx_dwconv_pre_bwd_drop: T <= 8192, a noise index within 32 bits and p in [0, 1)");
+  const DwDrop drop{(float4*)dzd, (uint32_t)sid_base, key, p};
+  dwconv_pre_bwd_launch<3, DW_PRE_GELU, true>(g, x, z, w, dz, dw, db, B, T, C, stream, drop);
+  ASRX_LAUNCHED("asrx_dwconv_pre_bwd_drop");
+}
+
 int asrx_bn_fwd(const float* x, const float* w, const float* b, float* y, float* mean, float* rstd, int64_t B,
                 int64_t T, int64_t C, float eps, int use_batch_stats, hipStream_t stream) {
   if (B * T == 0) return 0;
@@ -2946,19 +2988,30 @@
   return C % 4 == 0 && (al & 15) == 0 && B * T * C < (1LL << 31);
 }
 
-int asrx_bn_silu_fwd(const float* x, const float* w, const float* b, float* y, float* mean, float* rstd, int64_t B,
-                     int64_t T, int64_t C, float eps, int use_batch_stats, hipStream_t stream) {
+static int bn_silu_fwd(const char* name, const float* x, const float* w, const float* b, void* y, int out_bf16,
+                       float* mean, float* rstd, int64_t B, int64_t T, int64_t C, float eps, int use_batch_stats,
+                       hipStream_t stream) {
   if (B * T == 0) return 0;
   ASRX_REQUIRE(bn_silu_vec_ok({x, w, b, y, mean, rstd}, B, T, C),
-               "asrx_bn_silu_fwd: needs C %% 4 == 0, 16-byte aligned tensors and B*T*C < 2^31");
+               "%s: needs C %% 4 == 0, 16-byte aligned tensors and B*T*C < 2^31", name);
   const int C4 = (int)(C / 4);
   if (use_batch_stats)
     bn_stats4_kernel<<<(unsigned)(B * ((C4 + 31) / 32)), 1024, 0, stream>>>((const float4*)x, mean, rstd, (int)T, C4,
                                                                            eps);
   const int64_t n4 = B * T * C4;
-  LAUNCH_EW(bn_silu_apply4_kernel, n4, (const float4*)x, mean, rstd, w, b, (float4*)y, (uint32_t)n4, (uint32_t)C4,
-            (uint32_t)T, use_batch_stats);
-  ASRX_LAUNCHED("asrx_bn_silu_fwd");
+  LAUNCH_EW(bn_silu_apply4_kernel, n4, (const float4*)x, mean, rstd, w, b, out_bf16 ? nullptr : (float4*)y,
+            (uint32_t)n4, (uint32_t)C4, (uint32_t)T, use_batch_stats, out_bf16 ? (uint2*)y : nullptr);
+  return asrx::check_launch(name);
+}
+
+int asrx_bn_silu_fwd(const float* x, const float* w, const float* b, float* y, float* mean, float* rstd, int64_t B,
+                     int64_t T, int64_t C, float eps, int use_batch_stats, hipStream_t stream) {
+  return bn_silu_fwd("asrx_bn_silu_fwd", x, w, b, y, 0, mean, rstd, B, T, C, eps, use_batch_stats, stream);
+}
+
+int asrx_bn_silu_fwd_bf16(const float* x, const float* w, const float* b, unsigned short* y, float* mean, float* rstd,
+                          int64_t B, int64_t T, int64_t C, float eps, int use_batch_stats, hipStream_t stream) {
+  return bn_silu_fwd("asrx_bn_silu_fwd_bf16", x, w, b, y, 1, mean, rstd, B, T, C, eps, use_batch_stats, stream);
 }
 
 int asrx_bn_silu_bwd(const float* g, const float* x, const float* mean, const float* rstd, const float* w,
@@ -3039,3 +3092,16 @@
 }
 
 ASRX_NOISE_EPOCH_SETTER(asrx_set_noise_epoch_rowops)
+
+extern "C" const uint32_t* asrx_noise_epoch_addr_rowops(void) {
+  static std::atomic<const uint32_t*> known[64];
+  int dev = -1;
+  if (hipGetDevice(&dev) != hipSuccess) return nullptr;
+  const bool slot = dev >= 0 && dev < 64;
+  if (slot)
+    if (const uint32_t* q = known[dev].load(std::memory_order_acquire)) return q;
+  void* p = nullptr;
+  if (hipGetSymbolAddress(&p, HIP_SYMBOL(asrx::g_noise_epoch)) != hipSuccess) return nullptr;
+  if (slot) known[dev].store(static_cast<const uint32_t*>(p), std::memory_order_release);
+  return static_cast<const uint32_t*>(p);
+}
diff --git a/include/asrx.h b/include/asrx.h
--- a/include/asrx.h
+++ b/include/asrx.h
@@ -364,6 +364,9 @@
                     int64_t T, int64_t C, int64_t K, asrx_stream_t stream);
 int asrx_dwconv_pre_bwd(const float* g, const float* x, const float* z, const float* w, float* dz, float* dw,
                         float* db, int64_t B, int64_t T, int64_t C, int64_t K, int pre, asrx_stream_t stream);
+int asrx_dwconv_pre_bwd_drop(const float* g, const float* x, const float* z, const float* w, float* dz, float* dzd,
+                             float* dw, float* db, int64_t B, int64_t T, int64_t C, int64_t K, int pre,
+                             int64_t sid_base, uint32_t key, float p, asrx_stream_t stream);
 int asrx_bn_fwd(const float* x, const float* w, const float* b, float* y, float* mean, float* rstd, int64_t B,
                 int64_t T, int64_t C, float eps, int use_batch_stats, asrx_stream_t stream);
 int asrx_bn_bwd(const float* g, const float* x, const float* mean, const float* rstd, const float* w, float* sg_ws,
@@ -371,6 +374,8 @@
                 asrx_stream_t stream);
 int asrx_bn_silu_fwd(const float* x, const float* w, const float* b, float* y, float* mean, float* rstd, int64_t B,
                      int64_t T, int64_t C, float eps, int use_batch_stats, asrx_stream_t stream);
+int asrx_bn_silu_fwd_bf16(const float* x, const float* w, const float* b, unsigned short* y, float* mean, float* rstd,
+                          int64_t B, int64_t T, int64_t C, float eps, int use_batch_stats, asrx_stream_t stream);
 int asrx_bn_silu_bwd(const float* g, const float* x, const float* mean, const float* rstd, const float* w,
                      const float* b, float* sg_ws, float* sgx_ws, float* dx, float* dw, float* db, int64_t B,
                      int64_t T, int64_t C, asrx_stream_t stream);
@@ -430,6 +435,9 @@
 int asrx_gemm_wn_res(const float* A, int64_t lda, const unsigned short* W, int64_t ldw, float* C, int64_t ldc,
                      const float* bias, const float* R, int64_t ldr, int64_t M, int64_t N, int64_t K, int nj,
                      asrx_stream_t stream);
+int asrx_gemm_dropres(const void* A, int a_bf16, int64_t lda, const unsigned short* W, int64_t ldw, float* C,
+                      int64_t ldc, const float* bias, const float* R, int64_t ldr, int64_t T, int64_t sid_base,
+                      uint32_t key, float p, int64_t M, int64_t N, int64_t K, int nj, asrx_stream_t stream);
 int asrx_act_bwd_bias(const float* g, const float* z, unsigned short* gz, float* db, int64_t rows, int64_t N, int act,
                       asrx_stream_t stream);
 int asrx_wgrad_bf16_ab(const void* A, int64_t lda, const void* B, int b_bf16, int64_t ldb, float* C, int64_t ldc,
```

New measurement: 5655 audio-sec/sec, median of 6. No clear change (+0.6%).
